# Crowsinc/LiveVisionKit

Measured on AMD Instinct MI355X. Metric: stabilized frames/sec (one 4K YUV420 stream per GPU, steady state), higher is better.
Workload: dtype f32

## Files before the change

### include/lvk_hip.h

```cpp
#ifndef LVK_HIP_H
#define LVK_HIP_H

#include <stdint.h>
#include <stddef.h>

#ifdef __cplusplus
extern "C" {
#endif

#define LVK_HIP_OK              0
#define LVK_HIP_ERR_ARG        -1
#define LVK_HIP_ERR_RUNTIME    -2
#define LVK_HIP_ERR_NO_DEVICE  -3

typedef struct lvk_hip_ctx lvk_hip_ctx;


int  lvk_hip_ctx_create(int device, lvk_hip_ctx** out);
int  lvk_hip_ctx_create_on_stream(int device, void* hip_stream, lvk_hip_ctx** out);
void lvk_hip_ctx_destroy(lvk_hip_ctx* ctx);
int  lvk_hip_sync(lvk_hip_ctx* ctx);
void* lvk_hip_stream(lvk_hip_ctx* ctx);
const char* lvk_hip_last_error(lvk_hip_ctx* ctx);
const char* lvk_hip_version(void);
#define LVK_HIP_ABI_VERSION 12
int  lvk_hip_abi_version(void);
int  lvk_hip_device_count(void);
int  lvk_hip_device_usable(int device);

int  lvk_hip_ctx_wait(lvk_hip_ctx* ctx, lvk_hip_ctx* producer);

int lvk_hip_malloc(lvk_hip_ctx* ctx, size_t bytes, void** d_ptr);
int lvk_hip_free(lvk_hip_ctx* ctx, void* d_ptr);
int lvk_hip_trim(lvk_hip_ctx* ctx);
int lvk_hip_upload(lvk_hip_ctx* ctx, void* d_dst, const void* h_src, size_t bytes);
int lvk_hip_download(lvk_hip_ctx* ctx, void* h_dst, const void* d_src, size_t bytes);

int  lvk_hip_host_malloc(lvk_hip_ctx* ctx, size_t bytes, void** h_ptr);
int  lvk_hip_host_free(lvk_hip_ctx* ctx, void* h_ptr);


int lvk_hip_remap_homography(lvk_hip_ctx* ctx,
                             const void* d_src, int src_step, int src_rows, int src_cols,
                             void* d_dst, int dst_step, int dst_rows, int dst_cols,
                             int off_x, int off_y, const float H[9], const uint8_t bg[3], int yuv);

int lvk_hip_remap_mesh(lvk_hip_ctx* ctx,
                       const void* d_src, int src_step, int src_rows, int src_cols,
                       void* d_dst, int dst_step,
                       const float* mesh, int mesh_rows, int mesh_cols, const uint8_t bg[3], int yuv);

int lvk_hip_remap_map(lvk_hip_ctx* ctx, const void* d_src, int src_step, int rows, int cols, void* d_dst, int dst_step,
                      const void* d_map, int map_step, const uint8_t bg[3], int yuv);

#define LVK_REMAP_EXACT 0
#define LVK_REMAP_1LSB  1
int lvk_hip_set_remap_precision(lvk_hip_ctx* ctx, int precision);
int lvk_hip_get_remap_precision(lvk_hip_ctx* ctx);

int lvk_hip_upscale(lvk_hip_ctx* ctx, const void* d_src, int src_step, int src_rows, int src_cols,
                    void* d_dst, int dst_step, int dst_rows, int dst_cols, int yuv);

int lvk_hip_sharpen(lvk_hip_ctx* ctx, const void* d_src, int src_step, int rows, int cols, void* d_dst, int dst_step, float sharpness);

typedef struct lvk_camera_params { double fx, fy, cx, cy, k1, k2, p1, p2, k3; } lvk_camera_params;
int lvk_hip_lens_map_create(lvk_hip_ctx* ctx, const lvk_camera_params* params, int rows, int cols, void** d_map, int view_xywh[4]);
int lvk_hip_lens_map_destroy(lvk_hip_ctx* ctx, void* d_map);
int lvk_hip_warpmesh_apply_lens(lvk_hip_ctx* ctx, const void* d_src, int src_step, int rows, int cols, void* d_dst, int dst_step,
                                const float* mesh, int mesh_rows, int mesh_cols, const uint8_t bg[3], int yuv, const lvk_camera_params* lens);
int lvk_hip_lens_undistort_points(lvk_hip_ctx* ctx, const lvk_camera_params* params, int rows, int cols, double sx, double sy,
                                  const float* pts, int n, float* out);

int lvk_hip_warpmesh_apply_yuv420(lvk_hip_ctx* ctx, const void* d_src, int src_step, int rows, int cols,
                                  void* o_y, int oy_step, void* o_u, int ou_step, void* o_v, int ov_step, int nv12,
                                  const float* mesh, int mesh_rows, int mesh_cols, const uint8_t bg[3]);

int lvk_hip_warpmesh_apply(lvk_hip_ctx* ctx,
                           const void* d_src, int src_step, int rows, int cols,
                           void* d_dst, int dst_step,
                           const float* mesh, int mesh_rows, int mesh_cols, const uint8_t bg[3], int yuv);

int lvk_hip_ingest_yuv420(lvk_hip_ctx* ctx, const void* d_y, int y_step, const void* d_u, int u_step, const void* d_v, int v_step, int nv12,
                          int rows, int cols, void* d_dst, int dst_step);
int lvk_hip_egress_yuv420(lvk_hip_ctx* ctx, const void* d_src, int src_step, int rows, int cols,
                          void* d_y, int y_step, void* d_u, int u_step, void* d_v, int v_step, int nv12);

#define LVK_VIDEO_FORMAT_I420 1
#define LVK_VIDEO_FORMAT_NV12 2
#define LVK_VIDEO_FORMAT_YVYU 3
#define LVK_VIDEO_FORMAT_YUY2 4
#define LVK_VIDEO_FORMAT_UYVY 5
#define LVK_VIDEO_FORMAT_RGBA 6
#define LVK_VIDEO_FORMAT_BGRA 7
#define LVK_VIDEO_FORMAT_BGRX 8
#define LVK_VIDEO_FORMAT_Y800 9
#define LVK_VIDEO_FORMAT_I444 10
#define LVK_VIDEO_FORMAT_BGR3 11
#define LVK_VIDEO_FORMAT_I422 12
#define LVK_VIDEO_FORMAT_I40A 13
#define LVK_VIDEO_FORMAT_I42A 14
#define LVK_VIDEO_FORMAT_YUVA 15
#define LVK_VIDEO_FORMAT_AYUV 16
int lvk_hip_ingest_obs(lvk_hip_ctx* ctx, int video_format, const void* const d_planes[3], const int steps[3], int rows, int cols, void* d_dst, int dst_step);
int lvk_hip_egress_obs(lvk_hip_ctx* ctx, int video_format, const void* d_src, int src_step, int rows, int cols, void* const d_planes[3], const int steps[3]);
int lvk_hip_obs_frame_format(int video_format);

typedef struct lvk_stab_settings
{
    int detection_width, detection_height;
    int detection_regions_x, detection_regions_y;
    int force_detection;
    float max_feature_density, min_feature_density, accumulation_rate;
    int track_local_motions;
    float temporal_smoothing, local_smoothing;
    int min_motion_samples;
    float acceptance_threshold, uniformity_threshold;
    int predictive_samples;
    float corrective_limit_x, corrective_limit_y;
    float smoothing_steps, response_rate;
    int motion_width, motion_height;
    float background[3];
    int crop_to_stable_region, stabilize_output;
    float min_scene_quality, min_tracking_quality;
} lvk_stab_settings;

typedef struct lvk_stab_stats
{
    float tracking_stability;
    float scene_quality, trust;
    float distribution;
    int n_detected, n_matched, n_tracked, frame_delay;
    double smoothing_factor;
    double homography[9];
} lvk_stab_stats;

#define LVK_FORMAT_BGR 0
#define LVK_FORMAT_BGRA 1
#define LVK_FORMAT_RGB 2
#define LVK_FORMAT_RGBA 3
#define LVK_FORMAT_YUV 4
#define LVK_FORMAT_GRAY 5

typedef struct lvk_hip_stab lvk_hip_stab;

void lvk_stab_default_settings(lvk_stab_settings* s);
int  lvk_hip_stab_create(lvk_hip_ctx* ctx, const lvk_stab_settings* settings, lvk_hip_stab** out);
void lvk_hip_stab_destroy(lvk_hip_stab* stab);
int  lvk_hip_stab_configure(lvk_hip_stab* stab, const lvk_stab_settings* settings);
int  lvk_hip_stab_restart(lvk_hip_stab* stab);
int  lvk_hip_stab_draw_trackers(lvk_hip_stab* stab);
int  lvk_hip_stab_draw_motion_mesh(lvk_hip_stab* stab);
int  lvk_hip_draw_grid(lvk_hip_ctx* ctx, void* d_dst, int dst_step, int rows, int cols, int grid_w, int grid_h, const uint8_t colour[3], int thickness);
int  lvk_hip_draw_crosses(lvk_hip_ctx* ctx, void* d_dst, int dst_step, int rows, int cols, const float* pts_xy, int n,
                          float scale_x, float scale_y, const uint8_t colour[3], int cross_size, int thickness);
int  lvk_hip_draw_points(lvk_hip_ctx* ctx, void* d_dst, int dst_step, int rows, int cols, const float* pts_xy, int n, float scale_x, float scale_y,
                         const uint8_t colour[3], int point_size);
int  lvk_hip_draw_rect(lvk_hip_ctx* ctx, void* d_dst, int dst_step, int rows, int cols, const int rect_xywh[4], const uint8_t colour[3], int thickness);
int  lvk_hip_draw_text(lvk_hip_ctx* ctx, void* d_dst, int dst_step, int rows, int cols, const char* text, int x, int y, const uint8_t colour[3],
                       int scale, int thickness);
int  lvk_hip_stab_set_lens(lvk_hip_stab* stab, const lvk_camera_params* params);
int  lvk_hip_stab_reset_context(lvk_hip_stab* stab);
int  lvk_hip_stab_ready(const lvk_hip_stab* stab);
int  lvk_hip_stab_frame_delay(const lvk_hip_stab* stab);
int  lvk_hip_stab_stable_region(const lvk_hip_stab* stab, int rows, int cols, int rect_xywh[4]);

typedef struct lvk_frame_info { int rows, cols, format; } lvk_frame_info;
int  lvk_hip_stab_next_output(const lvk_hip_stab* stab, int rows, int cols, int format, lvk_frame_info* out);
int  lvk_hip_stab_push(lvk_hip_stab* stab, const void* d_frame, int step, int rows, int cols, uint64_t timestamp, int format,
                       void* d_out, int out_step, int out_rows, int* produced, uint64_t* out_timestamp, const void** released,
                       lvk_frame_info* emitted);

int  lvk_hip_stab_push_yuv420(lvk_hip_stab* stab, const void* d_y, int y_step, const void* d_u, int u_step, const void* d_v, int v_step, int nv12,
                              int rows, int cols, uint64_t timestamp,
                              void* o_y, int oy_step, void* o_u, int ou_step, void* o_v, int ov_step, int o_rows,
                              int* produced, uint64_t* out_timestamp, lvk_frame_info* emitted);
int  lvk_hip_stab_push_obs(lvk_hip_stab* stab, int video_format, const void* const d_planes[3], const int steps[3], int rows, int cols, uint64_t timestamp,
                           void* const o_planes[3], const int o_steps[3], int o_rows, int* produced, uint64_t* out_timestamp, lvk_frame_info* emitted);

int  lvk_hip_stab_push_yuv420_host(lvk_hip_stab* stab, const void* h_y, int y_step, const void* h_u, int u_step, const void* h_v, int v_step, int nv12,
                                   int rows, int cols, uint64_t timestamp,
                                   void* oh_y, int oy_step, void* oh_u, int ou_step, void* oh_v, int ov_step, int o_rows,
                                   int* produced, uint64_t* out_timestamp, lvk_frame_info* emitted);
int  lvk_hip_stab_push_obs_host(lvk_hip_stab* stab, int video_format,
                                const void* const h_planes[3], const int steps[3], int rows, int cols, uint64_t timestamp,
                                void* const oh_planes[3], const int o_steps[3], int o_rows,
                                int* produced, uint64_t* out_timestamp, lvk_frame_info* emitted);
int  lvk_hip_stab_prefetch_yuv420_host(lvk_hip_stab* stab, const void* h_y, int y_step, const void* h_u, int u_step, const void* h_v, int v_step,
                                       int nv12, int rows, int cols);
int  lvk_hip_stab_prefetch_cancel(lvk_hip_stab* stab);
int  lvk_hip_stab_set_overlap(lvk_hip_stab* stab, int enable);
int  lvk_hip_stab_set_bulk_context(lvk_hip_stab* stab, lvk_hip_ctx* bulk);
void* lvk_hip_stab_output_stream(lvk_hip_stab* stab);
int  lvk_hip_stab_set_remap_precision(lvk_hip_stab* stab, int precision);
int  lvk_hip_stab_get_remap_precision(const lvk_hip_stab* stab);


typedef struct lvk_deblock_settings
{
    uint32_t detection_levels;
    uint32_t block_size;
    uint32_t filter_size;
    float filter_scaling;
} lvk_deblock_settings;

typedef struct lvk_hip_deblock lvk_hip_deblock;

void lvk_hip_deblock_default_settings(lvk_deblock_settings* s);
int  lvk_hip_deblock_create(lvk_hip_ctx* ctx, const lvk_deblock_settings* settings, lvk_hip_deblock** out);
int  lvk_hip_deblock_configure(lvk_hip_deblock* deb, const lvk_deblock_settings* settings);
void lvk_hip_deblock_destroy(lvk_hip_deblock* deb);
int  lvk_hip_deblock_apply(lvk_hip_deblock* deb, void* d_frame, int step, int rows, int cols, int format, int region_xywh[4]);
int  lvk_hip_deblock_draw_influence(const lvk_hip_deblock* deb, void* d_frame, int step, int rows, int cols, int format);
int  lvk_hip_deblock_filter_region(const lvk_hip_deblock* deb, int region_xywh[4]);

int  lvk_hip_cas(lvk_hip_ctx* ctx, const void* d_src, int src_step, int rows, int cols, int format, void* d_dst, int dst_step, float sharpness);

int  lvk_hip_reformat(lvk_hip_ctx* ctx, const void* d_src, int src_step, int rows, int cols, int src_format, void* d_dst, int dst_step,
                      int dst_format);

int  lvk_hip_fsr_easu(lvk_hip_ctx* ctx, const void* d_src, int src_step, int rows, int cols, int format, const int region_xywh[4], void* d_dst,
                      int dst_step, int out_rows, int out_cols);
int  lvk_hip_fsr_geometry(int rows, int cols, int out_rows, int out_cols, float multiplier, int maintain_aspect_ratio, const int crop_ltrb[4],
                          int region_xywh[4], int out_rows_cols[2], int* skip);
int  lvk_hip_text_size(const char* text, int scale, int thickness, int wh[2], int* baseline);



int  lvk_hip_stab_prefetch(lvk_hip_stab* stab, const void* d_frame, int step, int rows, int cols, int format);
int  lvk_hip_stab_prefetch_yuv420(lvk_hip_stab* stab, const void* d_y, int y_step, const void* d_u, int u_step, const void* d_v, int v_step,
                                  int nv12, int rows, int cols);
long long lvk_hip_stab_lookahead_frames(lvk_hip_stab* stab);

int lvk_hip_remap_homography_gray(lvk_hip_ctx* ctx, const void* d_src, int src_step, int src_rows, int src_cols,
                                  void* d_dst, int dst_step, int dst_rows, int dst_cols, int off_x, int off_y, const float H[9], uint8_t bg);
int lvk_hip_remap_mesh_gray(lvk_hip_ctx* ctx, const void* d_src, int src_step, int src_rows, int src_cols, void* d_dst, int dst_step,
                            const float* mesh, int mesh_rows, int mesh_cols, uint8_t bg);
int lvk_hip_remap_map_gray(lvk_hip_ctx* ctx, const void* d_src, int src_step, int rows, int cols, void* d_dst, int dst_step,
                           const void* d_map, int map_step, uint8_t bg);
int lvk_hip_warpmesh_apply_gray(lvk_hip_ctx* ctx, const void* d_src, int src_step, int rows, int cols, void* d_dst, int dst_step,
                                const float* mesh, int mesh_rows, int mesh_cols, uint8_t bg);
int lvk_hip_warpmesh_apply_lens_gray(lvk_hip_ctx* ctx, const void* d_src, int src_step, int rows, int cols, void* d_dst, int dst_step,
                                     const float* mesh, int mesh_rows, int mesh_cols, uint8_t bg, const lvk_camera_params* lens);
int  lvk_hip_stab_push_gray(lvk_hip_stab* stab, const void* d_frame, int step, int rows, int cols, uint64_t timestamp,
                            void* d_out, int out_step, int out_rows, int* produced, uint64_t* out_timestamp, const void** released,
                            lvk_frame_info* emitted);
int  lvk_hip_stab_push_gray_host(lvk_hip_stab* stab, const void* h_frame, int step, int rows, int cols, uint64_t timestamp,
                                 void* oh_out, int out_step, int out_rows, int* produced, uint64_t* out_timestamp, lvk_frame_info* emitted);

int lvk_hip_remap_homography_c4(lvk_hip_ctx* ctx, const void* d_src, int src_step, int src_rows, int src_cols,
                                void* d_dst, int dst_step, int dst_rows, int dst_cols, int off_x, int off_y, const float H[9], const uint8_t bg[4]);
int lvk_hip_remap_mesh_c4(lvk_hip_ctx* ctx, const void* d_src, int src_step, int src_rows, int src_cols, void* d_dst, int dst_step,
                          const float* mesh, int mesh_rows, int mesh_cols, const uint8_t bg[4]);
int lvk_hip_remap_map_c4(lvk_hip_ctx* ctx, const void* d_src, int src_step, int rows, int cols, void* d_dst, int dst_step,
                         const void* d_map, int map_step, const uint8_t bg[4]);
int lvk_hip_warpmesh_apply_c4(lvk_hip_ctx* ctx, const void* d_src, int src_step, int rows, int cols, void* d_dst, int dst_step,
                              const float* mesh, int mesh_rows, int mesh_cols, const uint8_t bg[4]);
int lvk_hip_warpmesh_apply_lens_c4(lvk_hip_ctx* ctx, const void* d_src, int src_step, int rows, int cols, void* d_dst, int dst_step,
                                   const float* mesh, int mesh_rows, int mesh_cols, const uint8_t bg[4], const lvk_camera_params* lens);
int  lvk_hip_stab_set_background_alpha(lvk_hip_stab* stab, int alpha);
int  lvk_hip_stab_push_c4(lvk_hip_stab* stab, const void* d_frame, int step, int rows, int cols, uint64_t timestamp, int format,
                          void* d_out, int out_step, int out_rows, int* produced, uint64_t* out_timestamp, const void** released,
                          lvk_frame_info* emitted);
int  lvk_hip_stab_push_c4_host(lvk_hip_stab* stab, const void* h_frame, int step, int rows, int cols, uint64_t timestamp, int format,
                               void* oh_out, int out_step, int out_rows, int* produced, uint64_t* out_timestamp, lvk_frame_info* emitted);

int lvk_hip_upscale_gray(lvk_hip_ctx* ctx, const void* d_src, int src_step, int src_rows, int src_cols, void* d_dst, int dst_step, int dst_rows, int dst_cols);
int lvk_hip_upscale_c4(lvk_hip_ctx* ctx, const void* d_src, int src_step, int src_rows, int src_cols, void* d_dst, int dst_step, int dst_rows, int dst_cols);
int lvk_hip_sharpen_gray(lvk_hip_ctx* ctx, const void* d_src, int src_step, int rows, int cols, void* d_dst, int dst_step, float sharpness);
int lvk_hip_sharpen_c4(lvk_hip_ctx* ctx, const void* d_src, int src_step, int rows, int cols, void* d_dst, int dst_step, float sharpness);

int lvk_hip_cas_gray(lvk_hip_ctx* ctx, const void* d_src, int src_step, int rows, int cols, void* d_dst, int dst_step, float sharpness);
int lvk_hip_fsr_easu_gray(lvk_hip_ctx* ctx, const void* d_src, int src_step, int rows, int cols, const int region_xywh[4],
                          void* d_dst, int dst_step, int out_rows, int out_cols);
int lvk_hip_fsr_easu_gray_path(int rw, int rh, int out_rows, int out_cols);


#define LVK_SCHED_PUSH_FREE_RUNNING   0
#define LVK_SCHED_PUSH_SYNCHRONISED   1
#define LVK_SCHED_INGEST_ON_TRACKER   2
#define LVK_SCHED_INGEST_ON_BULK      3
#define LVK_SCHED_INGEST_INLINE       4
#define LVK_SCHED_REMAP_PERSISTENT    5
#define LVK_SCHED_REMAP_FULL          6
#define LVK_SCHED_WAIT_SIGNAL_WORD    7
#define LVK_SCHED_WAIT_EVENT          8
#define LVK_SCHED_WAIT_WORD_TIMEOUT   9
#define LVK_SCHED_COUNT              10
int  lvk_hip_stab_schedule_counters(lvk_hip_stab* stab, long long out[LVK_SCHED_COUNT], int reset);

int  lvk_hip_stab_get_stats(const lvk_hip_stab* stab, lvk_stab_stats* out);
int  lvk_hip_stab_detector_frames(const lvk_hip_stab* stab, long long* on_device, long long* on_host);
int  lvk_hip_stab_get_meshes(const lvk_hip_stab* stab, float* motion, float* correction, int cap_floats);
int  lvk_hip_stab_get_features(const lvk_hip_stab* stab, float* xy_resp_age, int cap);


#define LVK_STAGE_DOWNSCALE 0
#define LVK_STAGE_PYRAMID   1
#define LVK_STAGE_FAST      2
#define LVK_STAGE_PYRLK     3
#define LVK_STAGE_MOTION    4
#define LVK_STAGE_REMAP     5
#define LVK_STAGE_INGEST    6
#define LVK_STAGE_EGRESS    7
#define LVK_STAGE_COUNT     8
int  lvk_hip_stab_set_profiling(lvk_hip_stab* stab, int enable);
int  lvk_hip_stab_get_profile(lvk_hip_stab* stab, double total_ms[LVK_STAGE_COUNT], long long launches[LVK_STAGE_COUNT]);

int lvk_hip_native_rcp(lvk_hip_ctx* ctx, const float* d_in, float* d_out, size_t n);

typedef struct lvk_hip_mesh_solver lvk_hip_mesh_solver;
int  lvk_hip_mesh_solver_create(lvk_hip_ctx* ctx, int cols, int rows, float gen_region_w, float gen_region_h,
                                float temporal_smoothing, float local_smoothing, int max_points, lvk_hip_mesh_solver** out);
void lvk_hip_mesh_solver_destroy(lvk_hip_mesh_solver* solver);
int  lvk_hip_mesh_solver_reset(lvk_hip_mesh_solver* solver);
int  lvk_hip_mesh_solver_solve(lvk_hip_mesh_solver* solver, const float* tracked, const float* matched, int n, float region_w, float region_h,
                               float temporal_now, float threshold, uint8_t* inliers, float* offsets);

int lvk_hip_luma_area_resize(lvk_hip_ctx* ctx, const void* d_src, int src_step, int pix_stride, int channel,
                             int srows, int scols, void* d_dst, int dst_step, int drows, int dcols);

int lvk_hip_pyr_down(lvk_hip_ctx* ctx, const void* d_src, int src_step, int rows, int cols, void* d_dst, int dst_step);
int lvk_hip_scharr(lvk_hip_ctx* ctx, const void* d_src, int src_step, int rows, int cols, void* d_dst);

int lvk_hip_build_pyramid(lvk_hip_ctx* ctx, const void* d_img, int step, int rows, int cols, int max_level, int win_w, int win_h,
                          uint8_t* levels, int16_t* derivs, int* level_rows, int* level_cols);

int lvk_hip_fast_detect(lvk_hip_ctx* ctx, const void* d_img, int step, int rows, int cols,
                        const int* regions, int nregions, uint32_t* out, int cap, int* counts);

int lvk_hip_pyrlk(lvk_hip_ctx* ctx, const void* d_prev, int prev_step, const void* d_next, int next_step, int rows, int cols,
                  const float* prev_pts, int n, float* next_pts, uint8_t* status,
                  int win_w, int win_h, int max_level, int max_count, double epsilon, double min_eig_threshold);

int lvk_hip_estimate_global_motion(lvk_hip_ctx* ctx, const float* pts1, const float* pts2, int n, double threshold,
                                   double region_w, double region_h, int full_homography, double H[9], uint8_t* mask);

int lvk_hip_estimate_global_motion_lo(lvk_hip_ctx* ctx, const float* pts1, const float* pts2, int n, double threshold,
                                      double region_w, double region_h, int full_homography, int lo_mode, double H[9], uint8_t* mask,
                                      int lo_info[2]);

int lvk_hip_fast_filter(lvk_hip_ctx* ctx, const float* prev, const float* matched, const uint8_t* status, int n, float* out_prev, float* out_matched);

#define LVK_TRACK_CHAIN_GUARD 64
#define LVK_TRACK_CHAIN_FILL  0xA5
typedef struct lvk_track_chain_desc
{
    const float* prev; const float* matched; const uint8_t* status; const float* und;
    const void* d_prev_img; int prev_step; const void* d_next_img; int next_step; int rows, cols;
    int win_w, win_h, max_level, max_count; double epsilon, min_eig;
    const lvk_camera_params* lens; int lens_rows, lens_cols; double lens_sx, lens_sy;
    int n_bound, count_on_device, n_word;
    int full, model_on_device, full_word;
    int separate_compact, host_signal;
    double threshold; int region_w, region_h;
} lvk_track_chain_desc;
typedef struct lvk_track_chain_result
{
    double H[9]; int rc, signalled, count_dev, count_host;
    uint8_t* mask; float* pairs_dev; float* mirror_matched; uint8_t* mirror_status;
    float* next_pts; uint8_t* flow_status; float* flow_und;
} lvk_track_chain_result;
int lvk_hip_track_chain(lvk_hip_ctx* ctx, const lvk_track_chain_desc* desc, lvk_track_chain_result* result);

int lvk_hip_deblock_get_grid(lvk_hip_deblock* deb, uint8_t* mean, uint8_t* grid, float* keep_block, int capacity, int extent_xy[2]);


int lvk_hip_cas_const(float sharpness, float* peak);

int lvk_hip_cvt_code_target(int code, int src_format, int dcn);

int lvk_hip_fsr_easu_const(int rw, int rh, int W, int H, int ow, int oh, float con[16]);

int lvk_hip_fsr_easu_path(int rw, int rh, int out_rows, int out_cols);

enum
{
    LVK_AREA_PATH_FAST_DW_8x8_C3_BGR = 0, LVK_AREA_PATH_FAST_DW_8x8_C3_RGB = 1, LVK_AREA_PATH_FAST_DW_4x4_C3_BGR = 2, LVK_AREA_PATH_FAST_DW_4x4_C3_RGB = 3,
    LVK_AREA_PATH_FAST_DW_8x8_C3 = 4, LVK_AREA_PATH_FAST_DW_4x4_C3 = 5, LVK_AREA_PATH_FAST_DW_8x8_C1 = 6, LVK_AREA_PATH_FAST_DW_4x4_C1 = 7,
    LVK_AREA_PATH_FAST = 8, LVK_AREA_PATH_TILE_4 = 9, LVK_AREA_PATH_TILE_8 = 10, LVK_AREA_PATH_TAPS_4 = 11, LVK_AREA_PATH_TAPS_8 = 12,
    LVK_AREA_PATH_GENERAL = 13, LVK_AREA_PATH_ENLARGE = 14, LVK_AREA_PATH_COUNT = 15
};
int lvk_hip_area_resize_path(lvk_hip_ctx* ctx, const void* d_src, int src_step, int pix_stride, int channel,
                             int srows, int scols, int drows, int dcols);

int lvk_hip_remap_map_yuv420(lvk_hip_ctx* ctx, const void* d_src, int src_step, int rows, int cols,
                             void* o_y, int oy_step, void* o_u, int ou_step, void* o_v, int ov_step, int nv12,
                             const void* d_map, int map_step, const uint8_t bg[3]);
typedef struct lvk_hip_lens lvk_hip_lens;
int  lvk_hip_lens_create(lvk_hip_ctx* ctx, const lvk_camera_params* profile , int test_mode, lvk_hip_lens** out);
int  lvk_hip_lens_configure(lvk_hip_lens* lens, const lvk_camera_params* profile, int test_mode);
void lvk_hip_lens_destroy(lvk_hip_lens* lens);
int  lvk_hip_lens_view(lvk_hip_lens* lens, int rows, int cols, int view_xywh[4]);
int  lvk_hip_lens_apply(lvk_hip_lens* lens, void* d_src, int src_step, int rows, int cols, int format, void* d_dst, int dst_step);
int  lvk_hip_lens_apply_gray(lvk_hip_lens* lens, const void* d_src, int src_step, int rows, int cols, void* d_dst, int dst_step);
int  lvk_hip_lens_apply_c4(lvk_hip_lens* lens, const void* d_src, int src_step, int rows, int cols, int format, void* d_dst, int dst_step);
int  lvk_hip_lens_apply_yuv420(lvk_hip_lens* lens, const void* d_y, int y_step, const void* d_u, int u_step, const void* d_v, int v_step,
                               void* o_y, int oy_step, void* o_u, int ou_step, void* o_v, int ov_step, int rows, int cols, int nv12);

#ifdef __cplusplus
}
#endif

#include "lvk_hip_scaling_420.h"
#include "lvk_hip_deblock_420.h"
#include "lvk_hip_deblock_px.h"
#endif
```

### livevisionkit_amd/_native.py

```python
import ctypes
import os

_HERE = os.path.dirname(os.path.abspath(__file__))
LIB_PATH = os.environ.get("LVK_HIP_LIB") or os.path.join(_HERE, "liblvk_hip.so")

_c = ctypes
_P = _c.c_void_p
_SIG = {
    "lvk_hip_ctx_create": (_c.c_int, [_c.c_int, _c.POINTER(_P)]),
    "lvk_hip_ctx_create_on_stream": (_c.c_int, [_c.c_int, _P, _c.POINTER(_P)]),
    "lvk_hip_ctx_destroy": (None, [_P]),
    "lvk_hip_sync": (_c.c_int, [_P]),
    "lvk_hip_stream": (_P, [_P]),
    "lvk_hip_last_error": (_c.c_char_p, [_P]),
    "lvk_hip_version": (_c.c_char_p, []),
    "lvk_hip_abi_version": (_c.c_int, []),
    "lvk_hip_device_count": (_c.c_int, []),
    "lvk_hip_device_usable": (_c.c_int, [_c.c_int]),
    "lvk_hip_malloc": (_c.c_int, [_P, _c.c_size_t, _c.POINTER(_P)]),
    "lvk_hip_free": (_c.c_int, [_P, _P]),
    "lvk_hip_trim": (_c.c_int, [_P]),
    "lvk_hip_ctx_wait": (_c.c_int, [_P, _P]),
    "lvk_hip_upload": (_c.c_int, [_P, _P, _P, _c.c_size_t]),
    "lvk_hip_download": (_c.c_int, [_P, _P, _P, _c.c_size_t]),
    "lvk_hip_remap_homography": (_c.c_int, [_P, _P, _c.c_int, _c.c_int, _c.c_int, _P, _c.c_int, _c.c_int, _c.c_int,
                                            _c.c_int, _c.c_int, _c.POINTER(_c.c_float), _c.POINTER(_c.c_uint8), _c.c_int]),
    "lvk_hip_remap_mesh": (_c.c_int, [_P, _P, _c.c_int, _c.c_int, _c.c_int, _P, _c.c_int,
                                      _c.POINTER(_c.c_float), _c.c_int, _c.c_int, _c.POINTER(_c.c_uint8), _c.c_int]),
    "lvk_hip_remap_map": (_c.c_int, [_P, _P, _c.c_int, _c.c_int, _c.c_int, _P, _c.c_int, _P, _c.c_int, _c.POINTER(_c.c_uint8), _c.c_int]),
    "lvk_hip_remap_homography_gray": (_c.c_int, [_P, _P, _c.c_int, _c.c_int, _c.c_int, _P, _c.c_int, _c.c_int, _c.c_int,
                                                 _c.c_int, _c.c_int, _c.POINTER(_c.c_float), _c.c_uint8]),
    "lvk_hip_remap_mesh_gray": (_c.c_int, [_P, _P, _c.c_int, _c.c_int, _c.c_int, _P, _c.c_int, _c.POINTER(_c.c_float), _c.c_int, _c.c_int, _c.c_uint8]),
    "lvk_hip_remap_map_gray": (_c.c_int, [_P, _P, _c.c_int, _c.c_int, _c.c_int, _P, _c.c_int, _P, _c.c_int, _c.c_uint8]),
    "lvk_hip_warpmesh_apply_gray": (_c.c_int, [_P, _P, _c.c_int, _c.c_int, _c.c_int, _P, _c.c_int, _c.POINTER(_c.c_float), _c.c_int, _c.c_int, _c.c_uint8]),
    "lvk_hip_warpmesh_apply_lens_gray": (_c.c_int, [_P, _P, _c.c_int, _c.c_int, _c.c_int, _P, _c.c_int, _c.POINTER(_c.c_float), _c.c_int, _c.c_int, _c.c_uint8, _P]),
    "lvk_hip_stab_push_gray": (_c.c_int, [_P, _P, _c.c_int, _c.c_int, _c.c_int, _c.c_uint64, _P, _c.c_int, _c.c_int,
                                          _c.POINTER(_c.c_int), _c.POINTER(_c.c_uint64), _c.POINTER(_P), _P]),
    "lvk_hip_stab_push_gray_host": (_c.c_int, [_P, _P, _c.c_int, _c.c_int, _c.c_int, _c.c_uint64, _P, _c.c_int, _c.c_int,
                                               _c.POINTER(_c.c_int), _c.POINTER(_c.c_uint64), _P]),
    "lvk_hip_set_remap_precision": (_c.c_int, [_P, _c.c_int]),
    "lvk_hip_get_remap_precision": (_c.c_int, [_P]),
    "lvk_hip_stab_set_remap_precision": (_c.c_int, [_P, _c.c_int]),
    "lvk_hip_stab_get_remap_precision": (_c.c_int, [_P]),
    "lvk_hip_remap_homography_c4": (_c.c_int, [_P, _P, _c.c_int, _c.c_int, _c.c_int, _P, _c.c_int, _c.c_int, _c.c_int,
                                               _c.c_int, _c.c_int, _c.POINTER(_c.c_float), _c.POINTER(_c.c_uint8)]),
    "lvk_hip_remap_mesh_c4": (_c.c_int, [_P, _P, _c.c_int, _c.c_int, _c.c_int, _P, _c.c_int, _c.POINTER(_c.c_float), _c.c_int, _c.c_int, _c.POINTER(_c.c_uint8)]),
    "lvk_hip_remap_map_c4": (_c.c_int, [_P, _P, _c.c_int, _c.c_int, _c.c_int, _P, _c.c_int, _P, _c.c_int, _c.POINTER(_c.c_uint8)]),
    "lvk_hip_warpmesh_apply_c4": (_c.c_int, [_P, _P, _c.c_int, _c.c_int, _c.c_int, _P, _c.c_int, _c.POINTER(_c.c_float), _c.c_int, _c.c_int, _c.POINTER(_c.c_uint8)]),
    "lvk_hip_warpmesh_apply_lens_c4": (_c.c_int, [_P, _P, _c.c_int, _c.c_int, _c.c_int, _P, _c.c_int, _c.POINTER(_c.c_float), _c.c_int, _c.c_int, _c.POINTER(_c.c_uint8), _P]),
    "lvk_hip_stab_set_background_alpha": (_c.c_int, [_P, _c.c_int]),
    "lvk_hip_stab_push_c4": (_c.c_int, [_P, _P, _c.c_int, _c.c_int, _c.c_int, _c.c_uint64, _c.c_int, _P, _c.c_int, _c.c_int,
                                        _c.POINTER(_c.c_int), _c.POINTER(_c.c_uint64), _c.POINTER(_P), _P]),
    "lvk_hip_stab_push_c4_host": (_c.c_int, [_P, _P, _c.c_int, _c.c_int, _c.c_int, _c.c_uint64, _c.c_int, _P, _c.c_int, _c.c_int,
                                             _c.POINTER(_c.c_int), _c.POINTER(_c.c_uint64), _P]),
    "lvk_hip_upscale": (_c.c_int, [_P, _P, _c.c_int, _c.c_int, _c.c_int, _P, _c.c_int, _c.c_int, _c.c_int, _c.c_int]),
    "lvk_hip_sharpen": (_c.c_int, [_P, _P, _c.c_int, _c.c_int, _c.c_int, _P, _c.c_int, _c.c_float]),
    "lvk_hip_upscale_gray": (_c.c_int, [_P, _P, _c.c_int, _c.c_int, _c.c_int, _P, _c.c_int, _c.c_int, _c.c_int]),
    "lvk_hip_upscale_c4": (_c.c_int, [_P, _P, _c.c_int, _c.c_int, _c.c_int, _P, _c.c_int, _c.c_int, _c.c_int]),
    "lvk_hip_sharpen_gray": (_c.c_int, [_P, _P, _c.c_int, _c.c_int, _c.c_int, _P, _c.c_int, _c.c_float]),
    "lvk_hip_sharpen_c4": (_c.c_int, [_P, _P, _c.c_int, _c.c_int, _c.c_int, _P, _c.c_int, _c.c_float]),
    "lvk_hip_native_rcp": (_c.c_int, [_P, _P, _P, _c.c_size_t]),
    "lvk_hip_mesh_solver_create": (_c.c_int, [_P, _c.c_int, _c.c_int, _c.c_float, _c.c_float, _c.c_float, _c.c_float, _c.c_int, _c.POINTER(_P)]),
    "lvk_hip_mesh_solver_destroy": (None, [_P]),
    "lvk_hip_mesh_solver_reset": (_c.c_int, [_P]),
    "lvk_hip_mesh_solver_solve": (_c.c_int, [_P, _c.POINTER(_c.c_float), _c.POINTER(_c.c_float), _c.c_int, _c.c_float, _c.c_float, _c.c_float, _c.c_float,
                                             _c.POINTER(_c.c_uint8), _c.POINTER(_c.c_float)]),
    "lvk_hip_lens_map_create": (_c.c_int, [_P, _P, _c.c_int, _c.c_int, _c.POINTER(_P), _c.POINTER(_c.c_int)]),
    "lvk_hip_lens_map_destroy": (_c.c_int, [_P, _P]),
    "lvk_hip_warpmesh_apply_lens": (_c.c_int, [_P, _P, _c.c_int, _c.c_int, _c.c_int, _P, _c.c_int, _c.POINTER(_c.c_float), _c.c_int, _c.c_int, _c.POINTER(_c.c_uint8), _c.c_int, _P]),
    "lvk_hip_lens_undistort_points": (_c.c_int, [_P, _P, _c.c_int, _c.c_int, _c.c_double, _c.c_double, _c.POINTER(_c.c_float), _c.c_int, _c.POINTER(_c.c_float)]),
    "lvk_hip_stab_set_lens": (_c.c_int, [_P, _P]),
    "lvk_hip_stab_output_stream": (_P, [_P]),
    "lvk_hip_fast_filter": (_c.c_int, [_P, _c.POINTER(_c.c_float), _c.POINTER(_c.c_float), _c.POINTER(_c.c_uint8), _c.c_int, _c.POINTER(_c.c_float), _c.POINTER(_c.c_float)]),
    "lvk_hip_stab_draw_trackers": (_c.c_int, [_P]),
    "lvk_hip_stab_draw_motion_mesh": (_c.c_int, [_P]),
    "lvk_hip_draw_grid": (_c.c_int, [_P, _P, _c.c_int, _c.c_int, _c.c_int, _c.c_int, _c.c_int, _c.POINTER(_c.c_uint8), _c.c_int]),
    "lvk_hip_draw_crosses": (_c.c_int, [_P, _P, _c.c_int, _c.c_int, _c.c_int, _c.POINTER(_c.c_float), _c.c_int, _c.c_float, _c.c_float,
                                        _c.POINTER(_c.c_uint8), _c.c_int, _c.c_int]),
    "lvk_hip_draw_points": (_c.c_int, [_P, _P, _c.c_int, _c.c_int, _c.c_int, _c.POINTER(_c.c_float), _c.c_int, _c.c_float, _c.c_float,
                                       _c.POINTER(_c.c_uint8), _c.c_int]),
    "lvk_hip_draw_rect": (_c.c_int, [_P, _P, _c.c_int, _c.c_int, _c.c_int, _c.POINTER(_c.c_int), _c.POINTER(_c.c_uint8), _c.c_int]),
    "lvk_hip_draw_text": (_c.c_int, [_P, _P, _c.c_int, _c.c_int, _c.c_int, _c.c_char_p, _c.c_int, _c.c_int, _c.POINTER(_c.c_uint8), _c.c_int, _c.c_int]),
    "lvk_hip_text_size": (_c.c_int, [_c.c_char_p, _c.c_int, _c.c_int, _c.POINTER(_c.c_int), _c.POINTER(_c.c_int)]),
    "lvk_hip_warpmesh_apply_yuv420": (_c.c_int, [_P, _P, _c.c_int, _c.c_int, _c.c_int, _P, _c.c_int, _P, _c.c_int, _P, _c.c_int, _c.c_int,
                                                 _c.POINTER(_c.c_float), _c.c_int, _c.c_int, _c.POINTER(_c.c_uint8)]),
    "lvk_hip_warpmesh_apply": (_c.c_int, [_P, _P, _c.c_int, _c.c_int, _c.c_int, _P, _c.c_int,
                                          _c.POINTER(_c.c_float), _c.c_int, _c.c_int, _c.POINTER(_c.c_uint8), _c.c_int]),
    "lvk_hip_luma_area_resize": (_c.c_int, [_P, _P, _c.c_int, _c.c_int, _c.c_int, _c.c_int, _c.c_int, _P, _c.c_int, _c.c_int, _c.c_int]),
    "lvk_hip_pyr_down": (_c.c_int, [_P, _P, _c.c_int, _c.c_int, _c.c_int, _P, _c.c_int]),
    "lvk_hip_scharr": (_c.c_int, [_P, _P, _c.c_int, _c.c_int, _c.c_int, _P]),
    "lvk_hip_build_pyramid": (_c.c_int, [_P, _P, _c.c_int, _c.c_int, _c.c_int, _c.c_int, _c.c_int, _c.c_int,
                                         _c.POINTER(_c.c_uint8), _c.POINTER(_c.c_int16), _c.POINTER(_c.c_int), _c.POINTER(_c.c_int)]),
    "lvk_hip_fast_detect": (_c.c_int, [_P, _P, _c.c_int, _c.c_int, _c.c_int, _c.POINTER(_c.c_int), _c.c_int,
                                       _c.POINTER(_c.c_uint32), _c.c_int, _c.POINTER(_c.c_int)]),
    "lvk_hip_pyrlk": (_c.c_int, [_P, _P, _c.c_int, _P, _c.c_int, _c.c_int, _c.c_int, _c.POINTER(_c.c_float), _c.c_int,
                                 _c.POINTER(_c.c_float), _c.POINTER(_c.c_uint8), _c.c_int, _c.c_int, _c.c_int, _c.c_int,
                                 _c.c_double, _c.c_double]),
    "lvk_hip_ingest_yuv420": (_c.c_int, [_P, _P, _c.c_int, _P, _c.c_int, _P, _c.c_int, _c.c_int, _c.c_int, _c.c_int, _P, _c.c_int]),
    "lvk_hip_egress_yuv420": (_c.c_int, [_P, _P, _c.c_int, _c.c_int, _c.c_int, _P, _c.c_int, _P, _c.c_int, _P, _c.c_int, _c.c_int]),
    "lvk_hip_ingest_obs": (_c.c_int, [_P, _c.c_int, _P * 3, _c.c_int * 3, _c.c_int, _c.c_int, _P, _c.c_int]),
    "lvk_hip_egress_obs": (_c.c_int, [_P, _c.c_int, _P, _c.c_int, _c.c_int, _c.c_int, _P * 3, _c.c_int * 3]),
    "lvk_hip_obs_frame_format": (_c.c_int, [_c.c_int]),
    "lvk_hip_estimate_global_motion": (_c.c_int, [_P, _c.POINTER(_c.c_float), _c.POINTER(_c.c_float), _c.c_int, _c.c_double,
                                                  _c.c_double, _c.c_double, _c.c_int, _c.POINTER(_c.c_double), _c.POINTER(_c.c_uint8)]),
    "lvk_hip_estimate_global_motion_lo": (_c.c_int, [_P, _c.POINTER(_c.c_float), _c.POINTER(_c.c_float), _c.c_int, _c.c_double,
                                                     _c.c_double, _c.c_double, _c.c_int, _c.c_int, _c.POINTER(_c.c_double), _c.POINTER(_c.c_uint8),
                                                     _c.POINTER(_c.c_int)]),
    "lvk_hip_track_chain": (_c.c_int, [_P, _P, _P]),
    "lvk_stab_default_settings": (None, [_P]),
    "lvk_hip_stab_create": (_c.c_int, [_P, _P, _c.POINTER(_P)]),
    "lvk_hip_stab_destroy": (None, [_P]),
    "lvk_hip_stab_configure": (_c.c_int, [_P, _P]),
    "lvk_hip_stab_restart": (_c.c_int, [_P]),
    "lvk_hip_stab_reset_context": (_c.c_int, [_P]),
    "lvk_hip_stab_ready": (_c.c_int, [_P]),
    "lvk_hip_stab_frame_delay": (_c.c_int, [_P]),
    "lvk_hip_stab_stable_region": (_c.c_int, [_P, _c.c_int, _c.c_int, _c.POINTER(_c.c_int)]),
    "lvk_hip_stab_next_output": (_c.c_int, [_P, _c.c_int, _c.c_int, _c.c_int, _P]),
    "lvk_hip_stab_push": (_c.c_int, [_P, _P, _c.c_int, _c.c_int, _c.c_int, _c.c_uint64, _c.c_int, _P, _c.c_int, _c.c_int,
                                     _c.POINTER(_c.c_int), _c.POINTER(_c.c_uint64), _c.POINTER(_P), _P]),
    "lvk_hip_stab_push_yuv420": (_c.c_int, [_P, _P, _c.c_int, _P, _c.c_int, _P, _c.c_int, _c.c_int, _c.c_int, _c.c_int, _c.c_uint64,
                                            _P, _c.c_int, _P, _c.c_int, _P, _c.c_int, _c.c_int, _c.POINTER(_c.c_int), _c.POINTER(_c.c_uint64), _P]),
    "lvk_hip_stab_push_obs": (_c.c_int, [_P, _c.c_int, _P * 3, _c.c_int * 3, _c.c_int, _c.c_int, _c.c_uint64, _P * 3, _c.c_int * 3, _c.c_int,
                                         _c.POINTER(_c.c_int), _c.POINTER(_c.c_uint64), _P]),
    "lvk_hip_stab_push_yuv420_host": (_c.c_int, [_P, _P, _c.c_int, _P, _c.c_int, _P, _c.c_int, _c.c_int, _c.c_int, _c.c_int, _c.c_uint64,
                                            _P, _c.c_int, _P, _c.c_int, _P, _c.c_int, _c.c_int, _c.POINTER(_c.c_int), _c.POINTER(_c.c_uint64), _P]),
    "lvk_hip_stab_push_obs_host": (_c.c_int, [_P, _c.c_int, _P * 3, _c.c_int * 3, _c.c_int, _c.c_int, _c.c_uint64, _P * 3, _c.c_int * 3, _c.c_int,
                                              _c.POINTER(_c.c_int), _c.POINTER(_c.c_uint64), _P]),
    "lvk_hip_stab_prefetch_yuv420_host": (_c.c_int, [_P, _P, _c.c_int, _P, _c.c_int, _P, _c.c_int, _c.c_int, _c.c_int, _c.c_int]),
    "lvk_hip_stab_prefetch_cancel": (_c.c_int, [_P]),
    "lvk_hip_stab_prefetch": (_c.c_int, [_P, _P, _c.c_int, _c.c_int, _c.c_int, _c.c_int]),
    "lvk_hip_stab_prefetch_yuv420": (_c.c_int, [_P, _P, _c.c_int, _P, _c.c_int, _P, _c.c_int, _c.c_int, _c.c_int, _c.c_int]),
    "lvk_hip_stab_lookahead_frames": (_c.c_longlong, [_P]),
    "lvk_hip_stab_schedule_counters": (_c.c_int, [_P, _c.POINTER(_c.c_longlong), _c.c_int]),
    "lvk_hip_stab_detector_frames": (_c.c_int, [_P, _c.POINTER(_c.c_longlong), _c.POINTER(_c.c_longlong)]),
    "lvk_hip_host_malloc": (_c.c_int, [_P, _c.c_size_t, _c.POINTER(_P)]),
    "lvk_hip_host_free": (_c.c_int, [_P, _P]),
    "lvk_hip_stab_get_stats": (_c.c_int, [_P, _P]),
    "lvk_hip_stab_get_meshes": (_c.c_int, [_P, _c.POINTER(_c.c_float), _c.POINTER(_c.c_float), _c.c_int]),
    "lvk_hip_stab_get_features": (_c.c_int, [_P, _c.POINTER(_c.c_float), _c.c_int]),
    "lvk_hip_stab_set_overlap": (_c.c_int, [_P, _c.c_int]),
    "lvk_hip_stab_set_bulk_context": (_c.c_int, [_P, _P]),
    "lvk_hip_stab_set_profiling": (_c.c_int, [_P, _c.c_int]),
    "lvk_hip_stab_get_profile": (_c.c_int, [_P, _c.POINTER(_c.c_double), _c.POINTER(_c.c_longlong)]),
    "lvk_hip_deblock_default_settings": (None, [_P]),
    "lvk_hip_deblock_create": (_c.c_int, [_P, _P, _c.POINTER(_P)]),
    "lvk_hip_deblock_configure": (_c.c_int, [_P, _P]),
    "lvk_hip_deblock_destroy": (None, [_P]),
    "lvk_hip_deblock_apply": (_c.c_int, [_P, _P, _c.c_int, _c.c_int, _c.c_int, _c.c_int, _c.POINTER(_c.c_int)]),
    "lvk_hip_deblock_draw_influence": (_c.c_int, [_P, _P, _c.c_int, _c.c_int, _c.c_int, _c.c_int]),
    "lvk_hip_deblock_filter_region": (_c.c_int, [_P, _c.POINTER(_c.c_int)]),
    "lvk_hip_deblock_get_grid": (_c.c_int, [_P, _c.POINTER(_c.c_uint8), _c.POINTER(_c.c_uint8), _c.POINTER(_c.c_float), _c.c_int, _c.POINTER(_c.c_int)]),
    "lvk_hip_cas": (_c.c_int, [_P, _P, _c.c_int, _c.c_int, _c.c_int, _c.c_int, _P, _c.c_int, _c.c_float]),
    "lvk_hip_cas_const": (_c.c_int, [_c.c_float, _c.POINTER(_c.c_float)]),
    "lvk_hip_reformat": (_c.c_int, [_P, _P, _c.c_int, _c.c_int, _c.c_int, _c.c_int, _P, _c.c_int, _c.c_int]),
    "lvk_hip_cvt_code_target": (_c.c_int, [_c.c_int, _c.c_int, _c.c_int]),
    "lvk_hip_fsr_easu": (_c.c_int, [_P, _P, _c.c_int, _c.c_int, _c.c_int, _c.c_int, _c.POINTER(_c.c_int), _P, _c.c_int, _c.c_int, _c.c_int]),
    "lvk_hip_fsr_geometry": (_c.c_int, [_c.c_int, _c.c_int, _c.c_int, _c.c_int, _c.c_float, _c.c_int, _c.POINTER(_c.c_int), _c.POINTER(_c.c_int),
                                        _c.POINTER(_c.c_int), _c.POINTER(_c.c_int)]),
    "lvk_hip_fsr_easu_const": (_c.c_int, [_c.c_int, _c.c_int, _c.c_int, _c.c_int, _c.c_int, _c.c_int, _c.POINTER(_c.c_float)]),
    "lvk_hip_fsr_easu_path": (_c.c_int, [_c.c_int, _c.c_int, _c.c_int, _c.c_int]),
    "lvk_hip_cas_gray": (_c.c_int, [_P, _P, _c.c_int, _c.c_int, _c.c_int, _P, _c.c_int, _c.c_float]),
    "lvk_hip_fsr_easu_gray": (_c.c_int, [_P, _P, _c.c_int, _c.c_int, _c.c_int, _c.POINTER(_c.c_int), _P, _c.c_int, _c.c_int, _c.c_int]),
    "lvk_hip_fsr_easu_gray_path": (_c.c_int, [_c.c_int, _c.c_int, _c.c_int, _c.c_int]),
    "lvk_hip_area_resize_path": (_c.c_int, [_P, _P, _c.c_int, _c.c_int, _c.c_int, _c.c_int, _c.c_int, _c.c_int, _c.c_int]),
    "lvk_hip_remap_map_yuv420": (_c.c_int, [_P, _P, _c.c_int, _c.c_int, _c.c_int, _P, _c.c_int, _P, _c.c_int, _P, _c.c_int, _c.c_int,
                                            _P, _c.c_int, _c.POINTER(_c.c_uint8)]),
    "lvk_hip_lens_create": (_c.c_int, [_P, _P, _c.c_int, _c.POINTER(_P)]),
    "lvk_hip_lens_configure": (_c.c_int, [_P, _P, _c.c_int]),
    "lvk_hip_lens_destroy": (None, [_P]),
    "lvk_hip_lens_view": (_c.c_int, [_P, _c.c_int, _c.c_int, _c.POINTER(_c.c_int)]),
    "lvk_hip_lens_apply": (_c.c_int, [_P, _P, _c.c_int, _c.c_int, _c.c_int, _c.c_int, _P, _c.c_int]),
    "lvk_hip_lens_apply_gray": (_c.c_int, [_P, _P, _c.c_int, _c.c_int, _c.c_int, _P, _c.c_int]),
    "lvk_hip_lens_apply_c4": (_c.c_int, [_P, _P, _c.c_int, _c.c_int, _c.c_int, _c.c_int, _P, _c.c_int]),
    "lvk_hip_lens_apply_yuv420": (_c.c_int, [_P, _P, _c.c_int, _P, _c.c_int, _P, _c.c_int, _P, _c.c_int, _P, _c.c_int, _P, _c.c_int,
                                             _c.c_int, _c.c_int, _c.c_int]),
}

_SIG_DEBLOCK_PX = {
    "lvk_hip_deblock_apply_gray": (_c.c_int, [_P, _P, _c.c_int, _c.c_int, _c.c_int, _c.POINTER(_c.c_int)]),
    "lvk_hip_deblock_apply_c4": (_c.c_int, [_P, _P, _c.c_int, _c.c_int, _c.c_int, _c.c_int, _c.POINTER(_c.c_int)]),
}

_SIG_DEBLOCK_420 = {
    "lvk_hip_deblock_apply_yuv420": (_c.c_int, [_P, _P, _c.c_int, _P, _c.c_int, _P, _c.c_int, _P, _c.c_int, _P, _c.c_int, _P, _c.c_int,
                                                _c.c_int, _c.c_int, _c.c_int, _c.POINTER(_c.c_int)]),
}

_SIG_SCALING_420 = {
    "lvk_hip_scale_yuv420": (_c.c_int, [_P, _P, _c.c_int, _P, _c.c_int, _P, _c.c_int, _c.c_int, _c.c_int,
                                        _P, _c.c_int, _P, _c.c_int, _P, _c.c_int, _c.c_int, _c.c_int, _c.c_int, _c.c_float]),
}

_lib = None


def symbols():
    return sorted(_SIG.keys())


def symbols_deblock_px():
    return sorted(_SIG_DEBLOCK_PX.keys())


def symbols_deblock_420():
    return sorted(_SIG_DEBLOCK_420.keys())


def symbols_scaling_420():
    return sorted(_SIG_SCALING_420.keys())


def load():
    global _lib
    if _lib is not None:
        return _lib
    if not os.path.exists(LIB_PATH):
        raise RuntimeError(
            f"{LIB_PATH} is missing: build it with `python -c 'import __graft_entry__ as g; g.build()'` "
            "(or `make -C livevisionkit_amd/csrc`). There is no CPU fallback.")
    import torch
    lib = ctypes.CDLL(LIB_PATH, mode=ctypes.RTLD_GLOBAL)
    for name, (res, args) in {**_SIG, **_SIG_DEBLOCK_PX, **_SIG_DEBLOCK_420, **_SIG_SCALING_420}.items():
        fn = getattr(lib, name)
        fn.restype = res
        fn.argtypes = args
    _lib = lib
    return lib
```

### livevisionkit_amd/context.py

```python
import ctypes

import numpy as np

from . import _native


class LvkHipError(RuntimeError):
    pass


def _f32(a):
    a = np.ascontiguousarray(a, dtype=np.float32)
    return a, a.ctypes.data_as(ctypes.POINTER(ctypes.c_float))


def _u8x3(bg):
    a = np.ascontiguousarray(bg, dtype=np.uint8).reshape(3)
    return a, a.ctypes.data_as(ctypes.POINTER(ctypes.c_uint8))


def _u8x4(bg):
    a = np.ascontiguousarray(bg, dtype=np.uint8).reshape(4)
    return a, a.ctypes.data_as(ctypes.POINTER(ctypes.c_uint8))


def _planes420_empty(rows, cols, nv12, device):
    import torch
    y = torch.empty((rows, cols), dtype=torch.uint8, device=device)
    u = torch.empty((rows // 2, cols // 2, 2) if nv12 else (rows // 2, cols // 2), dtype=torch.uint8, device=device)
    return (y, u) if nv12 else (y, u, torch.empty_like(u))


def _planes420_args(planes, nv12):
    a = []
    for p in planes[:2 if nv12 else 3]:
        a += [p.data_ptr(), p.stride(0)]
    return a + ([None, 0] if nv12 else [])


TRACK_CHAIN_GUARD = 64
TRACK_CHAIN_FILL = 0xA5


class TrackChainDesc(ctypes.Structure):
    _fields_ = [("prev", ctypes.POINTER(ctypes.c_float)), ("matched", ctypes.POINTER(ctypes.c_float)), ("status", ctypes.POINTER(ctypes.c_uint8)),
                ("und", ctypes.POINTER(ctypes.c_float)),
                ("d_prev_img", ctypes.c_void_p), ("prev_step", ctypes.c_int), ("d_next_img", ctypes.c_void_p), ("next_step", ctypes.c_int),
                ("rows", ctypes.c_int), ("cols", ctypes.c_int),
                ("win_w", ctypes.c_int), ("win_h", ctypes.c_int), ("max_level", ctypes.c_int), ("max_count", ctypes.c_int),
                ("epsilon", ctypes.c_double), ("min_eig", ctypes.c_double),
                ("lens", ctypes.c_void_p), ("lens_rows", ctypes.c_int), ("lens_cols", ctypes.c_int), ("lens_sx", ctypes.c_double), ("lens_sy", ctypes.c_double),
                ("n_bound", ctypes.c_int), ("count_on_device", ctypes.c_int), ("n_word", ctypes.c_int),
                ("full", ctypes.c_int), ("model_on_device", ctypes.c_int), ("full_word", ctypes.c_int),
                ("separate_compact", ctypes.c_int), ("host_signal", ctypes.c_int),
                ("threshold", ctypes.c_double), ("region_w", ctypes.c_int), ("region_h", ctypes.c_int)]


class TrackChainResult(ctypes.Structure):
    _fields_ = [("H", ctypes.c_double * 9), ("rc", ctypes.c_int), ("signalled", ctypes.c_int), ("count_dev", ctypes.c_int), ("count_host", ctypes.c_int),
                ("mask", ctypes.POINTER(ctypes.c_uint8)), ("pairs_dev", ctypes.POINTER(ctypes.c_float)), ("mirror_matched", ctypes.POINTER(ctypes.c_float)),
                ("mirror_status", ctypes.POINTER(ctypes.c_uint8)),
                ("next_pts", ctypes.POINTER(ctypes.c_float)), ("flow_status", ctypes.POINTER(ctypes.c_uint8)), ("flow_und", ctypes.POINTER(ctypes.c_float))]

REMAP_EXACT, REMAP_1LSB = 0, 1


def _remap_precision(precision):
    if isinstance(precision, str):
        return {"exact": REMAP_EXACT, "1lsb": REMAP_1LSB}.get(precision.lower(), -1)
    return int(precision)


class Context:

    def __init__(self, device=0, stream=None):
        import torch
        if not torch.cuda.is_available():
            raise LvkHipError("no GPU visible: the lvk HIP path has no CPU fallback")
        self.lib = _native.load()
        self.device = device
        torch.cuda.set_device(device)
        self._torch_stream = stream if stream is not None else torch.cuda.current_stream(device)
        handle = ctypes.c_void_p()
        rc = self.lib.lvk_hip_ctx_create_on_stream(device, ctypes.c_void_p(self._torch_stream.cuda_stream), ctypes.byref(handle))
        if rc != 0:
            raise LvkHipError(f"lvk_hip_ctx_create failed ({rc}): {self.lib.lvk_hip_last_error(None).decode()}")
        self.handle = handle

    def close(self):
        if getattr(self, "handle", None):
            self.lib.lvk_hip_ctx_destroy(self.handle)
            self.handle = None

    def __del__(self):
        try:
            self.close()
        except Exception:
            pass

    def _check(self, rc):
        if rc != 0:
            raise LvkHipError(f"lvk_hip call failed ({rc}): {self.lib.lvk_hip_last_error(self.handle).decode()}")

    def sync(self):
        self._check(self.lib.lvk_hip_sync(self.handle))

    def set_remap_precision(self, precision):
        self._check(self.lib.lvk_hip_set_remap_precision(self.handle, _remap_precision(precision)))

    @property
    def remap_precision(self):
        return self.lib.lvk_hip_get_remap_precision(self.handle)

    def remap_homography(self, src, H, bg=(255, 0, 255), yuv=True, out=None, dst_size=None, offset=(0, 0)):
        import torch
        rows, cols = src.shape[0], src.shape[1]
        drows, dcols = dst_size if dst_size is not None else (rows, cols)
        if out is None:
            out = torch.empty((drows, dcols, 3), dtype=torch.uint8, device=src.device)
        Ha, Hp = _f32(np.asarray(H, dtype=np.float32).reshape(9))
        bga, bgp = _u8x3(bg)
        self._check(self.lib.lvk_hip_remap_homography(
            self.handle, src.data_ptr(), src.stride(0), rows, cols, out.data_ptr(), out.stride(0), drows, dcols,
            offset[0], offset[1], Hp, bgp, 1 if yuv else 0))
        return out

    def remap_mesh(self, src, mesh, bg=(255, 0, 255), yuv=True, out=None):
        import torch
        rows, cols = src.shape[0], src.shape[1]
        if out is None:
            out = torch.empty((rows, cols, 3), dtype=torch.uint8, device=src.device)
        m = np.ascontiguousarray(mesh, dtype=np.float32)
        ma, mp = _f32(m)
        bga, bgp = _u8x3(bg)
        self._check(self.lib.lvk_hip_remap_mesh(
            self.handle, src.data_ptr(), src.stride(0), rows, cols, out.data_ptr(), out.stride(0),
            mp, m.shape[0], m.shape[1], bgp, 1 if yuv else 0))
        return out

    def warpmesh_apply(self, src, mesh, bg=(255, 0, 255), yuv=True, out=None):
        import torch
        rows, cols = src.shape[0], src.shape[1]
        if out is None:
            out = torch.empty((rows, cols, 3), dtype=torch.uint8, device=src.device)
        m = np.ascontiguousarray(mesh, dtype=np.float32)
        ma, mp = _f32(m)
        bga, bgp = _u8x3(bg)
        self._check(self.lib.lvk_hip_warpmesh_apply(
            self.handle, src.data_ptr(), src.stride(0), rows, cols, out.data_ptr(), out.stride(0),
            mp, m.shape[0], m.shape[1], bgp, 1 if yuv else 0))
        return out

    def _px_out(self, sfx, src, out, shape=None):
        import torch
        if sfx == "_gray" and src.dim() != 2:
            raise ValueError("a one-channel frame is a [rows, cols] uint8 tensor")
        if sfx == "_c4" and (src.dim() != 3 or src.shape[2] != 4):
            raise ValueError("a four-channel frame is a [rows, cols, 4] uint8 tensor")
        return out if out is not None else torch.empty(tuple(shape or src.shape[:2]) + tuple(src.shape[2:]), dtype=torch.uint8, device=src.device)

    def _px_call(self, name, sfx, src, out, bg, mid, tail=(), shape=None):
        out = self._px_out(sfx, src, out, shape)
        bga, bgp = (None, int(bg)) if sfx == "_gray" else _u8x4(bg)
        self._check(getattr(self.lib, "lvk_hip_" + name + sfx)(self.handle, src.data_ptr(), src.stride(0), src.shape[0], src.shape[1], out.data_ptr(), out.stride(0),
                                                               *mid, bgp, *tail))
        return out

    def _px_homography(self, sfx, src, H, bg, out, dst_size, offset):
        drows, dcols = dst_size if dst_size is not None else tuple(src.shape[:2])
        Ha, Hp = _f32(np.asarray(H, dtype=np.float32).reshape(9))
        return self._px_call("remap_homography", sfx, src, out, bg, (drows, dcols, offset[0], offset[1], Hp), shape=(drows, dcols))

    def _px_mesh(self, name, sfx, src, mesh, bg, out, lens=None):
        ma, mp = _f32(mesh)
        tail = () if lens is None else ((ctypes.c_double * 9)(*[float(v) for v in lens]),)
        return self._px_call(name, sfx, src, out, bg, (mp, ma.shape[0], ma.shape[1]), tail)

    def _px_map(self, sfx, src, offsets, bg, out):
        return self._px_call("remap_map", sfx, src, out, bg, (offsets.data_ptr(), offsets.stride(0) * 4))

    def remap_homography_gray(self, src, H, bg=0, out=None, dst_size=None, offset=(0, 0)):
        return self._px_homography("_gray", src, H, bg, out, dst_size, offset)

    def remap_mesh_gray(self, src, mesh, bg=0, out=None):
        return self._px_mesh("remap_mesh", "_gray", src, mesh, bg, out)

    def remap_map_gray(self, src, offsets, bg=0, out=None):
        return self._px_map("_gray", src, offsets, bg, out)

    def warpmesh_apply_gray(self, src, mesh, bg=0, out=None, lens=None):
        return self._px_mesh("warpmesh_apply" if lens is None else "warpmesh_apply_lens", "_gray", src, mesh, bg, out, lens)

    def remap_homography_c4(self, src, H, bg=(255, 0, 255, 255), out=None, dst_size=None, offset=(0, 0)):
        return self._px_homography("_c4", src, H, bg, out, dst_size, offset)

    def remap_mesh_c4(self, src, mesh, bg=(255, 0, 255, 255), out=None):
        return self._px_mesh("remap_mesh", "_c4", src, mesh, bg, out)

    def remap_map_c4(self, src, offsets, bg=(255, 0, 255, 255), out=None):
        return self._px_map("_c4", src, offsets, bg, out)

    def warpmesh_apply_c4(self, src, mesh, bg=(255, 0, 255, 255), out=None):
        return self._px_mesh("warpmesh_apply", "_c4", src, mesh, bg, out)

    def warpmesh_apply_lens_c4(self, src, mesh, lens, bg=(255, 0, 255, 255), out=None):
        return self._px_mesh("warpmesh_apply_lens", "_c4", src, mesh, bg, out, lens)

    def luma_area_resize(self, frame, drows, dcols, channel=0, out=None):
        import torch
        pix = frame.shape[2] if frame.dim() == 3 else 1
        if out is None:
            out = torch.empty((drows, dcols), dtype=torch.uint8, device=frame.device)
        self._check(self.lib.lvk_hip_luma_area_resize(self.handle, frame.data_ptr(), frame.stride(0), pix, channel,
                                                      frame.shape[0], frame.shape[1], out.data_ptr(), out.stride(0), drows, dcols))
        return out

    def area_resize_path(self, frame, drows, dcols, channel=0):
        pix = frame.shape[2] if frame.dim() == 3 else 1
        path = self.lib.lvk_hip_area_resize_path(self.handle, frame.data_ptr(), frame.stride(0), pix, channel, frame.shape[0], frame.shape[1], drows, dcols)
        self._check(min(path, 0))
        return path

    def pyr_down(self, img, out=None):
        import torch
        if out is None:
            out = torch.empty(((img.shape[0] + 1) // 2, (img.shape[1] + 1) // 2), dtype=torch.uint8, device=img.device)
        self._check(self.lib.lvk_hip_pyr_down(self.handle, img.data_ptr(), img.stride(0), img.shape[0], img.shape[1],
                                              out.data_ptr(), out.stride(0)))
        return out

    def scharr(self, img, out=None):
        import torch
        if out is None:
            out = torch.empty((img.shape[0], img.shape[1], 2), dtype=torch.int16, device=img.device)
        self._check(self.lib.lvk_hip_scharr(self.handle, img.data_ptr(), img.stride(0), img.shape[0], img.shape[1], out.data_ptr()))
        return out

    def build_pyramid(self, img, max_level=3, win=(11, 11)):
        rows, cols = img.shape
        lv = np.zeros(rows * cols * 2, np.uint8); dv = np.zeros(rows * cols * 4, np.int16)
        lr = np.zeros(8, np.int32); lc = np.zeros(8, np.int32)
        n = self.lib.lvk_hip_build_pyramid(self.handle, img.data_ptr(), img.stride(0), rows, cols, max_level, win[0], win[1],
                                           lv.ctypes.data_as(ctypes.POINTER(ctypes.c_uint8)), dv.ctypes.data_as(ctypes.POINTER(ctypes.c_int16)),
                                           lr.ctypes.data_as(ctypes.POINTER(ctypes.c_int)), lc.ctypes.data_as(ctypes.POINTER(ctypes.c_int)))
        self._check(min(n, 0))
        out, lo, do = [], 0, 0
        for i in range(n):
            r, c = int(lr[i]), int(lc[i])
            out.append((lv[lo:lo + r * c].reshape(r, c).copy(), dv[do:do + r * c * 2].reshape(r, c, 2).copy()))
            lo += r * c; do += r * c * 2
        return out

    def fast_detect(self, img, regions, cap=None):
        rg = np.ascontiguousarray(regions, dtype=np.int32).reshape(-1, 6)
        n = rg.shape[0]
        cap = cap or int(max(1, (rg[:, 2] * rg[:, 3]).max()))
        out = np.zeros((n, cap), np.uint32)
        counts = np.zeros(n, np.int32)
        self._check(self.lib.lvk_hip_fast_detect(self.handle, img.data_ptr(), img.stride(0), img.shape[0], img.shape[1],
                                                 rg.ctypes.data_as(ctypes.POINTER(ctypes.c_int)), n,
                                                 out.ctypes.data_as(ctypes.POINTER(ctypes.c_uint32)), cap,
                                                 counts.ctypes.data_as(ctypes.POINTER(ctypes.c_int))))
        res = []
        for i in range(n):
            e = out[i, :min(cap, counts[i])]
            res.append(np.stack([e & 0xFFF, (e >> 12) & 0xFFF, e >> 24], axis=1).astype(np.int32))
        return res, counts

    def pyrlk(self, prev, nxt, pts, win=(11, 11), max_level=3, max_count=5, epsilon=0.01, min_eig=1e-4):
        pts = np.ascontiguousarray(pts, np.float32).reshape(-1, 2)
        out = np.zeros_like(pts)
        st = np.zeros(len(pts), np.uint8)
        self._check(self.lib.lvk_hip_pyrlk(self.handle, prev.data_ptr(), prev.stride(0), nxt.data_ptr(), nxt.stride(0),
                                           prev.shape[0], prev.shape[1],
                                           pts.ctypes.data_as(ctypes.POINTER(ctypes.c_float)), len(pts),
                                           out.ctypes.data_as(ctypes.POINTER(ctypes.c_float)),
                                           st.ctypes.data_as(ctypes.POINTER(ctypes.c_uint8)),
                                           win[0], win[1], max_level, max_count, float(epsilon), float(min_eig)))
        return out, st

    def estimate_global_motion(self, p1, p2, threshold, region=(480, 270), full_homography=True):
        p1 = np.ascontiguousarray(p1, np.float32).reshape(-1, 2); p2 = np.ascontiguousarray(p2, np.float32).reshape(-1, 2)
        H = np.zeros(9, np.float64); mask = np.zeros(len(p1), np.uint8)
        rc = self.lib.lvk_hip_estimate_global_motion(self.handle, p1.ctypes.data_as(ctypes.POINTER(ctypes.c_float)),
                                                     p2.ctypes.data_as(ctypes.POINTER(ctypes.c_float)), len(p1), float(threshold),
                                                     float(region[0]), float(region[1]), 1 if full_homography else 0,
                                                     H.ctypes.data_as(ctypes.POINTER(ctypes.c_double)),
                                                     mask.ctypes.data_as(ctypes.POINTER(ctypes.c_uint8)))
        if rc in (-1, -2, -3):
            self._check(rc)
        return rc, H.reshape(3, 3), mask

    def estimate_global_motion_lo(self, p1, p2, threshold, lo_mode, region=(480, 270), full_homography=True):
        p1 = np.ascontiguousarray(p1, np.float32).reshape(-1, 2); p2 = np.ascontiguousarray(p2, np.float32).reshape(-1, 2)
        H = np.zeros(9, np.float64); mask = np.zeros(len(p1), np.uint8); info = (ctypes.c_int * 2)(-1, -1)
        rc = self.lib.lvk_hip_estimate_global_motion_lo(self.handle, p1.ctypes.data_as(ctypes.POINTER(ctypes.c_float)),
                                                        p2.ctypes.data_as(ctypes.POINTER(ctypes.c_float)), len(p1), float(threshold),
                                                        float(region[0]), float(region[1]), 1 if full_homography else 0, int(lo_mode),
                                                        H.ctypes.data_as(ctypes.POINTER(ctypes.c_double)),
                                                        mask.ctypes.data_as(ctypes.POINTER(ctypes.c_uint8)), info)
        if rc in (-1, -2, -3):
            self._check(rc)
        return rc, H.reshape(3, 3), mask, info[0], info[1]

    def ingest_yuv420(self, y, u, v=None, out=None):
        import torch
        rows, cols = y.shape
        if out is None:
            out = torch.empty((rows, cols, 3), dtype=torch.uint8, device=y.device)
        nv12 = v is None
        self._check(self.lib.lvk_hip_ingest_yuv420(self.handle, *_planes420_args((y, u, v), nv12), 1 if nv12 else 0, rows, cols, out.data_ptr(), out.stride(0)))
        return out

    def egress_yuv420(self, frame, nv12=False, out=None):
        rows, cols = frame.shape[:2]
        if out is None:
            out = _planes420_empty(rows, cols, nv12, frame.device)
        y, u, v = out if not nv12 else (out[0], out[1], None)
        self._check(self.lib.lvk_hip_egress_yuv420(self.handle, frame.data_ptr(), frame.stride(0), rows, cols, *_planes420_args((y, u, v), nv12), 1 if nv12 else 0))
        return (y, u) if nv12 else (y, u, v)

    VIDEO_FORMATS = {"I420": 1, "NV12": 2, "YVYU": 3, "YUY2": 4, "UYVY": 5, "RGBA": 6, "BGRA": 7, "BGRX": 8, "Y800": 9, "I444": 10, "BGR3": 11,
                     "I422": 12, "I40A": 13, "I42A": 14, "YUVA": 15, "AYUV": 16}

    def _obs_args(self, planes):
        import ctypes as c
        ptrs = (c.c_void_p * 3)(*[p.data_ptr() for p in planes] + [None] * (3 - len(planes)))
        steps = (c.c_int * 3)(*[p.stride(0) for p in planes] + [0] * (3 - len(planes)))
        return ptrs, steps

    def ingest_obs(self, fmt, planes, out=None):
        import torch
        rows, cols = planes[0].shape[:2]
        if out is None:
            out = torch.empty((rows, cols) if fmt == "Y800" else (rows, cols, 3), dtype=torch.uint8, device=planes[0].device)
        ptrs, steps = self._obs_args(planes)
        self._check(self.lib.lvk_hip_ingest_obs(self.handle, self.VIDEO_FORMATS[fmt], ptrs, steps, rows, cols, out.data_ptr(), out.stride(0)))
        return out

    def egress_obs(self, fmt, frame, planes):
        rows, cols = frame.shape[:2]
        ptrs, steps = self._obs_args(planes)
        self._check(self.lib.lvk_hip_egress_obs(self.handle, self.VIDEO_FORMATS[fmt], frame.data_ptr(), frame.stride(0), rows, cols, ptrs, steps))
        return planes

    def obs_frame_format(self, fmt):
        return self.lib.lvk_hip_obs_frame_format(self.VIDEO_FORMATS[fmt] if isinstance(fmt, str) else int(fmt))

    def remap_map(self, src, offsets, bg=(255, 0, 255), yuv=True, out=None):
        import torch
        rows, cols = src.shape[:2]
        if out is None:
            out = torch.empty_like(src)
        bga, bgp = _u8x3(bg)
        self._check(self.lib.lvk_hip_remap_map(self.handle, src.data_ptr(), src.stride(0), rows, cols, out.data_ptr(), out.stride(0),
                                               offsets.data_ptr(), offsets.stride(0) * 4, bgp, 1 if yuv else 0))
        return out

    def remap_map_yuv420(self, src, offsets, bg=(255, 0, 255), nv12=False, out=None):
        rows, cols = src.shape[0], src.shape[1]
        out = _planes420_empty(rows, cols, nv12, src.device) if out is None else tuple(out)
        bga, bgp = _u8x3(bg)
        self._check(self.lib.lvk_hip_remap_map_yuv420(self.handle, src.data_ptr(), src.stride(0), rows, cols, *_planes420_args(out, nv12), 1 if nv12 else 0,
                                                      offsets.data_ptr(), offsets.stride(0) * 4, bgp))
        return out

    def upscale(self, src, size, yuv=True, out=None):
        import torch
        rows, cols = src.shape[:2]
        if out is None:
            out = torch.empty((int(size[1]), int(size[0]), 3), dtype=torch.uint8, device=src.device)
        self._check(self.lib.lvk_hip_upscale(self.handle, src.data_ptr(), src.stride(0), rows, cols,
                                             out.data_ptr(), out.stride(0), out.shape[0], out.shape[1], 1 if yuv else 0))
        return out

    def sharpen(self, src, sharpness=0.7, out=None):
        import torch
        rows, cols = src.shape[:2]
        if out is None:
            out = torch.empty_like(src)
        self._check(self.lib.lvk_hip_sharpen(self.handle, src.data_ptr(), src.stride(0), rows, cols, out.data_ptr(), out.stride(0),
                                             float(sharpness)))
        return out

    def scale_yuv420(self, y, u, v=None, size=None, sharpness=0.8, out=None):
        rows, cols = y.shape
        w, h = (cols, rows) if size is None else (int(size[0]), int(size[1]))
        nv12 = v is None
        out = _planes420_empty(h, w, nv12, y.device) if out is None else tuple(out)
        self._check(self.lib.lvk_hip_scale_yuv420(self.handle, *_planes420_args((y, u, v), nv12), rows, cols, *_planes420_args(out, nv12),
                                                  h, w, 1 if nv12 else 0, float(sharpness)))
        return out

    def _px_upscale(self, sfx, src, size, out):
        out = self._px_out(sfx, src, out, (int(size[1]), int(size[0])))
        self._check(getattr(self.lib, "lvk_hip_upscale" + sfx)(self.handle, src.data_ptr(), src.stride(0), src.shape[0], src.shape[1],
                                                               out.data_ptr(), out.stride(0), out.shape[0], out.shape[1]))
        return out

    def _px_sharpen(self, sfx, src, sharpness, out):
        out = self._px_out(sfx, src, out)
        self._check(getattr(self.lib, "lvk_hip_sharpen" + sfx)(self.handle, src.data_ptr(), src.stride(0), src.shape[0], src.shape[1],
                                                               out.data_ptr(), out.stride(0), float(sharpness)))
        return out

    def upscale_gray(self, src, size, out=None):
        return self._px_upscale("_gray", src, size, out)

    def upscale_c4(self, src, size, out=None):
        return self._px_upscale("_c4", src, size, out)

    def sharpen_gray(self, src, sharpness=0.7, out=None):
        return self._px_sharpen("_gray", src, sharpness, out)

    def sharpen_c4(self, src, sharpness=0.7, out=None):
        return self._px_sharpen("_c4", src, sharpness, out)

    def mesh_solver(self, cols, rows, gen_region=(480, 270), temporal=1.0, local=20.0, max_points=4096):
        return MeshSolver(self, cols, rows, gen_region, temporal, local, max_points)

    def native_rcp(self, x):
        import torch
        x = x.contiguous()
        out = torch.empty_like(x)
        self._check(self.lib.lvk_hip_native_rcp(self.handle, x.data_ptr(), out.data_ptr(), x.numel()))
        return out

    def lens_map(self, params, rows, cols):
        import torch
        arr = (ctypes.c_double * 9)(*[float(v) for v in params])
        d = ctypes.c_void_p(); view = (ctypes.c_int * 4)()
        self._check(self.lib.lvk_hip_lens_map_create(self.handle, arr, rows, cols, ctypes.byref(d), view))
        tmp = np.zeros((rows, cols, 2), np.float32)
        self._check(self.lib.lvk_hip_download(self.handle, tmp.ctypes.data_as(ctypes.c_void_p), d, tmp.nbytes))
        self.sync()
        t = torch.from_numpy(tmp).to("cuda")
        self._check(self.lib.lvk_hip_lens_map_destroy(self.handle, d))
        return t, tuple(view)

    def warpmesh_apply_lens(self, src, mesh, params, bg=(255, 0, 255), yuv=True, out=None):
        import torch
        rows, cols = src.shape[0], src.shape[1]
        if out is None:
            out = torch.empty((rows, cols, 3), dtype=torch.uint8, device=src.device)
        m = np.ascontiguousarray(mesh, dtype=np.float32)
        ma, mp = _f32(m)
        bga, bgp = _u8x3(bg)
        arr = (ctypes.c_double * 9)(*[float(v) for v in params])
        self._check(self.lib.lvk_hip_warpmesh_apply_lens(self.handle, src.data_ptr(), src.stride(0), rows, cols, out.data_ptr(), out.stride(0),
                                                         mp, m.shape[0], m.shape[1], bgp, 1 if yuv else 0, arr))
        return out

    def lens_undistort_points(self, params, rows, cols, sx, sy, pts):
        p = np.ascontiguousarray(pts, np.float32).reshape(-1, 2)
        out = np.zeros_like(p)
        arr = (ctypes.c_double * 9)(*[float(v) for v in params])
        fp = ctypes.POINTER(ctypes.c_float)
        self._check(self.lib.lvk_hip_lens_undistort_points(self.handle, arr, rows, cols, float(sx), float(sy), p.ctypes.data_as(fp), len(p), out.ctypes.data_as(fp)))
        return out

    def draw_grid(self, frame, grid, colour, thickness=1):
        ca, cp = _u8x3(colour)
        self._check(self.lib.lvk_hip_draw_grid(self.handle, frame.data_ptr(), frame.stride(0), frame.shape[0], frame.shape[1], int(grid[0]), int(grid[1]), cp, thickness))
        return frame

    def draw_crosses(self, frame, points, colour, cross_size, thickness, scaling=(1.0, 1.0)):
        p = np.ascontiguousarray(points, np.float32).reshape(-1, 2)
        ca, cp = _u8x3(colour)
        self._check(self.lib.lvk_hip_draw_crosses(self.handle, frame.data_ptr(), frame.stride(0), frame.shape[0], frame.shape[1],
                                                  p.ctypes.data_as(ctypes.POINTER(ctypes.c_float)), len(p), float(scaling[0]), float(scaling[1]), cp,
                                                  int(cross_size), int(thickness)))
        return frame

    def fast_filter(self, prev, matched, status):
        a = np.ascontiguousarray(prev, np.float32).reshape(-1, 2); b = np.ascontiguousarray(matched, np.float32).reshape(-1, 2)
        st = np.ascontiguousarray(status, np.uint8).reshape(-1)
        oa = np.zeros_like(a); ob = np.zeros_like(b)
        fp = ctypes.POINTER(ctypes.c_float)
        m = self.lib.lvk_hip_fast_filter(self.handle, a.ctypes.data_as(fp), b.ctypes.data_as(fp), st.ctypes.data_as(ctypes.POINTER(ctypes.c_uint8)), len(a),
                                         oa.ctypes.data_as(fp), ob.ctypes.data_as(fp))
        if m < 0:
            self._check(m)
        return oa[:m], ob[:m]

    def track_chain(self, prev, matched=None, status=None, und=None, images=None, win=(11, 11), max_level=3, max_count=5, epsilon=0.01, min_eig=1e-4,
                    lens=None, threshold=3.0, region=(480, 270), full=True, full_word=None, n_word=None, separate_compact=False, host_signal=False):
        fp, bp = ctypes.POINTER(ctypes.c_float), ctypes.POINTER(ctypes.c_uint8)
        prev = np.ascontiguousarray(prev, np.float32).reshape(-1, 2)
        nb, G = len(prev), TRACK_CHAIN_GUARD
        d, r = TrackChainDesc(), TrackChainResult()
        keep = [prev]
        d.prev = prev.ctypes.data_as(fp)
        if images is None:
            matched = np.ascontiguousarray(matched, np.float32).reshape(nb, 2); status = np.ascontiguousarray(status, np.uint8).reshape(nb)
            keep += [matched, status]
            d.matched = matched.ctypes.data_as(fp); d.status = status.ctypes.data_as(bp)
            if und is not None:
                und = np.ascontiguousarray(und, np.float32).reshape(-1, 2)
                n_eff = nb if n_word is None else min(max(int(n_word), 0), nb)
                if len(und) != 2 * n_eff:
                    raise ValueError("und holds 2 x the effective count of positions (previous | matched)")
                keep.append(und)
                d.und = und.ctypes.data_as(fp)
        else:
            a, b = images
            keep += [a, b]
            d.d_prev_img = a.data_ptr(); d.prev_step = a.stride(0); d.d_next_img = b.data_ptr(); d.next_step = b.stride(0)
            d.rows, d.cols = a.shape[0], a.shape[1]
            d.win_w, d.win_h, d.max_level, d.max_count, d.epsilon, d.min_eig = win[0], win[1], max_level, max_count, float(epsilon), float(min_eig)
            if lens is not None:
                params, lrows, lcols, sx, sy = lens
                arr = (ctypes.c_double * 9)(*[float(v) for v in params])
                keep.append(arr)
                d.lens = ctypes.cast(arr, ctypes.c_void_p); d.lens_rows, d.lens_cols, d.lens_sx, d.lens_sy = int(lrows), int(lcols), float(sx), float(sy)
        d.n_bound = nb
        d.count_on_device, d.n_word = (0, 0) if n_word is None else (1, int(n_word))
        d.full = 1 if full else 0
        d.model_on_device, d.full_word = (0, 0) if full_word is None else (1, int(full_word))
        d.separate_compact = 1 if separate_compact else 0; d.host_signal = 1 if host_signal else 0
        d.threshold = float(threshold); d.region_w, d.region_h = int(region[0]), int(region[1])
        mask = np.zeros(nb, np.uint8); pairs = np.zeros((2, nb, 2), np.float32); mm = np.zeros((nb, 2), np.float32); ms = np.zeros(nb, np.uint8)
        r.mask = mask.ctypes.data_as(bp); r.pairs_dev = pairs.ctypes.data_as(fp); r.mirror_matched = mm.ctypes.data_as(fp); r.mirror_status = ms.ctypes.data_as(bp)
        out = {}
        if images is not None:
            nxt = np.zeros((nb + 2 * G, 2), np.float32); fst = np.zeros(nb + 2 * G, np.uint8); fund = np.zeros((2 * nb + 2 * G, 2), np.float32)
            r.next_pts = nxt.ctypes.data_as(fp); r.flow_status = fst.ctypes.data_as(bp); r.flow_und = fund.ctypes.data_as(fp)
            out.update(next_pts=nxt, flow_status=fst, flow_und=fund)
        self._check(self.lib.lvk_hip_track_chain(self.handle, ctypes.byref(d), ctypes.byref(r)))
        del keep
        out.update(H=np.array(r.H, np.float64).reshape(3, 3), rc=r.rc, signalled=r.signalled, count_dev=r.count_dev, count_host=r.count_host, mask=mask,
                   pairs_dev=pairs, mirror_matched=mm, mirror_status=ms)
        return out

    def warpmesh_apply_yuv420(self, src, mesh, bg=(255, 0, 255), nv12=False):
        rows, cols = src.shape[0], src.shape[1]
        out = _planes420_empty(rows, cols, nv12, src.device)
        m = np.ascontiguousarray(mesh, dtype=np.float32)
        ma, mp = _f32(m)
        bga, bgp = _u8x3(bg)
        self._check(self.lib.lvk_hip_warpmesh_apply_yuv420(self.handle, src.data_ptr(), src.stride(0), rows, cols, *_planes420_args(out, nv12), 1 if nv12 else 0,
                                                           mp, m.shape[0], m.shape[1], bgp))
        return out


class MeshSolver:

    def __init__(self, ctx, cols, rows, gen_region, temporal, local, max_points):
        self.ctx, self.cols, self.rows = ctx, cols, rows
        h = ctypes.c_void_p()
        ctx._check(ctx.lib.lvk_hip_mesh_solver_create(ctx.handle, cols, rows, float(gen_region[0]), float(gen_region[1]), float(temporal), float(local),
                                                      int(max_points), ctypes.byref(h)))
        self.handle = h

    def solve(self, tracked, matched, region=(480, 270), temporal=1.0, threshold=10.0):
        t = np.ascontiguousarray(tracked, np.float32).reshape(-1, 2); m = np.ascontiguousarray(matched, np.float32).reshape(-1, 2)
        inl = np.zeros(len(t), np.uint8); off = np.zeros((self.rows, self.cols, 2), np.float32)
        fp = ctypes.POINTER(ctypes.c_float)
        rc = self.ctx.lib.lvk_hip_mesh_solver_solve(self.handle, t.ctypes.data_as(fp), m.ctypes.data_as(fp), len(t), float(region[0]), float(region[1]),
                                                    float(temporal), float(threshold), inl.ctypes.data_as(ctypes.POINTER(ctypes.c_uint8)), off.ctypes.data_as(fp))
        if rc < 0:
            self.ctx._check(rc)
        return rc, inl, off

    def reset(self):
        self.ctx._check(self.ctx.lib.lvk_hip_mesh_solver_reset(self.handle))

    def close(self):
        if getattr(self, "handle", None):
            if getattr(self.ctx, "handle", None):
                self.ctx.lib.lvk_hip_mesh_solver_destroy(self.handle)
            self.handle = None
```

### livevisionkit_amd/csrc/lvk_hip_internal.hpp

```cpp
#pragma once

#include <hip/hip_runtime.h>
#include <cstdint>
#include <cstdio>
#include <string>
#include <vector>
#include <functional>
#include <map>
#include <set>
#include <mutex>
#include <utility>

#include "lvk_hip.h"
#include "planes420.hpp"

struct LinTabEntry { int s0, s1; float a0, a1; };
struct Lin8Entry { int s0, s1, a0, a1; };
struct AreaTabEntry { int si; float alpha; };
struct FastRegion { int x, y, w, h, threshold, active; };
constexpr int LVK_FAST_INLINE_REGIONS = 8;

constexpr int LVK_MAX_PYR_LEVELS = 8;
struct PyrLevel { const uint8_t* img; const short2* deriv; int rows, cols, step; };
struct PyrArgs { PyrLevel lv[LVK_MAX_PYR_LEVELS]; int nlevels; };

struct lvk_hip_ctx
{
    int remap_precision = LVK_REMAP_EXACT;
    int device = 0;
    int cu_count = 0;
    hipStream_t stream = nullptr;
    bool owns_stream = false;
    std::string last_error;

    static constexpr int kStageSlots = 16;
    static constexpr size_t kStageBytes = 64 * 1024;
    uint8_t* stage_host = nullptr;
    uint8_t* stage_dev = nullptr;
    hipEvent_t stage_done[kStageSlots] = {};
    int stage_next = 0;

    std::vector<hipStream_t> aux_streams;
    std::mutex aux_mutex;
    std::vector<std::pair<void*, std::function<int()>>> sync_hooks;

    std::mutex pool_mutex;
    std::multimap<size_t, void*> pool_free;
    std::map<void*, size_t> pool_sizes;
    std::set<void*> pool_cached;
    size_t pool_cached_bytes = 0;
    static constexpr size_t kPoolMaxCachedBytes = (size_t)4 << 30;

    std::vector<hipEvent_t> wait_events;

    std::map<std::tuple<int, int, int>, LinTabEntry*> lintabs;

    std::map<std::tuple<int, int, int>, Lin8Entry*> lin8tabs;

    struct AreaTabDev { int2* range = nullptr; AreaTabEntry* tab = nullptr; int max_taps = 0, span64 = 0, span4 = 0; };
    std::map<std::pair<int, int>, AreaTabDev> areatabs;
    std::map<std::pair<int, int>, int4*> enlargetabs;

    int fail(int code, const std::string& msg) { last_error = msg; if (code == LVK_HIP_ERR_RUNTIME) (void)hipGetLastError(); return code; }
};

struct lvk_device_guard
{
    int prev = -1; bool switched = false;
    explicit lvk_device_guard(const lvk_hip_ctx* ctx)
    {
        if (hipGetDevice(&prev) != hipSuccess) { (void)hipGetLastError(); prev = -1; }
        if (prev != ctx->device) switched = hipSetDevice(ctx->device) == hipSuccess;
    }
    ~lvk_device_guard() { if (switched && prev >= 0) (void)hipSetDevice(prev); }
    lvk_device_guard(const lvk_device_guard&) = delete;
    lvk_device_guard& operator=(const lvk_device_guard&) = delete;
};

#define LVK_HIP_ENTRY(ctx)                         \
    if (!(ctx)) return LVK_HIP_ERR_ARG;            \
    lvk_device_guard lvk_entry_device_guard(ctx)

#define LVK_HIP_CHECK(ctx, expr)                                                                      \
    do {                                                                                              \
        hipError_t _e = (expr);                                                                       \
        if (_e != hipSuccess)                                                                         \
        {                                                                                             \
            (void)hipGetLastError();    \
            return (ctx)->fail(LVK_HIP_ERR_RUNTIME, std::string(#expr) + ": " + hipGetErrorString(_e)); \
        }                                                                                             \
    } while (0)

#ifndef LVK_TRACKER_PRIO
#define LVK_TRACKER_PRIO 3
#endif
#define LVK_TRACKER_PRIORITY() __builtin_amdgcn_s_setprio(LVK_TRACKER_PRIO)

#if (defined(LVK_TIMELINE) || defined(LVK_RANSAC_TIMING) || defined(LVK_MESH_TIMING)) && !defined(LVK_PROBE_BUILD)
#error "instrumented build: pass -DLVK_PROBE_BUILD (scripts/variant_build.sh); never the library the tests and the bench load by default"
#endif

#ifdef LVK_TIMELINE
#define LVK_TL_SLOTS 4
#define LVK_TL_RING 8192
static __device__ unsigned lvk_tl_head[LVK_TL_SLOTS];
static __device__ unsigned long long lvk_tl_log[LVK_TL_SLOTS][LVK_TL_RING][2];
struct LvkTimelineScope
{
    int slot; bool sampled; unsigned long long t0;
    __device__ explicit LvkTimelineScope(int s) : slot(s), sampled(false), t0(0)
    {
        const unsigned total = gridDim.x * gridDim.y * gridDim.z;
        const unsigned b = (blockIdx.z * gridDim.y + blockIdx.y) * gridDim.x + blockIdx.x;
        sampled = threadIdx.x == 0 && threadIdx.y == 0 && ((b & 63u) == 63u || b == 0 || b == total - 1);
        if (sampled) t0 = (unsigned long long)wall_clock64();
    }
    __device__ ~LvkTimelineScope()
    {
        if (sampled)
        {
            const unsigned i = atomicAdd(&lvk_tl_head[slot], 1u) % LVK_TL_RING;
            lvk_tl_log[slot][i][0] = t0; lvk_tl_log[slot][i][1] = (unsigned long long)wall_clock64();
        }
    }
};
#define LVK_TL(slot) LvkTimelineScope lvk_tl_scope_(slot)
#define LVK_TL_EXPORT(unit)                                                                                     \
    extern "C" int lvk_tl_read_##unit(long long* out)                                                           \
    {                                                                                                           \
        unsigned idx[LVK_TL_SLOTS];                                                                             \
        if (hipDeviceSynchronize() != hipSuccess) return -1;                                                    \
        if (hipMemcpyFromSymbol(idx, HIP_SYMBOL(lvk_tl_head), sizeof(idx)) != hipSuccess) return -1;           \
        for (int s = 0; s < LVK_TL_SLOTS; s++) out[(size_t)s * (1 + 2 * LVK_TL_RING)] = idx[s];                 \
        for (int s = 0; s < LVK_TL_SLOTS; s++)                                                                  \
            if (hipMemcpyFromSymbol(out + (size_t)s * (1 + 2 * LVK_TL_RING) + 1, HIP_SYMBOL(lvk_tl_log), sizeof(long long) * 2 * LVK_TL_RING, \
                                    sizeof(long long) * 2 * LVK_TL_RING * s) != hipSuccess) return -1;         \
        return 0;                                                                                               \
    }
#else
#define LVK_TL(slot) do { } while (0)
#define LVK_TL_EXPORT(unit)
#endif

#define LVK_HIP_REQUIRE(ctx, cond)                                                                    \
    do { if (!(cond)) return (ctx)->fail(LVK_HIP_ERR_ARG, "pre-condition failed: " #cond); } while (0)

inline int lvk_format_channels(int format)
{
    switch (format)
    {
    case LVK_FORMAT_BGR: case LVK_FORMAT_RGB: case LVK_FORMAT_YUV: return 3;
    case LVK_FORMAT_BGRA: case LVK_FORMAT_RGBA: return 4;
    case LVK_FORMAT_GRAY: return 1;
    default: return 0;
    }
}

inline bool lvk_pitched_overlap(const void* a, int a_step, int a_rows, long long a_row_bytes, const void* b, int b_step, int b_rows, long long b_row_bytes)
{
    return yuv420::overlap(yuv420::span_of(a, a_step, a_rows, a_row_bytes), yuv420::span_of(b, b_step, b_rows, b_row_bytes));
}

int lvk_stage_params(lvk_hip_ctx* ctx, hipStream_t stream, const void* host, size_t bytes, void** d_out, int* slot = nullptr);
int lvk_stage_consumed(lvk_hip_ctx* ctx, int slot, hipStream_t stream);

int lvk_get_lintab(lvk_hip_ctx* ctx, int msize, int fsize, bool vertical, const LinTabEntry** d_out);

int lvk_get_areatab(lvk_hip_ctx* ctx, int ssize, int dsize, const int2** d_range, const AreaTabEntry** d_tab, int* max_taps = nullptr, int* span64 = nullptr, int* span4 = nullptr);

int lvk_launch_luma_area_resize(lvk_hip_ctx* ctx, const void* d_src, int src_step, int pix_stride, int channel,
                                int srows, int scols, void* d_dst, int dst_step, int drows, int dcols);
int lvk_launch_pyr_down(lvk_hip_ctx* ctx, const void* d_src, int src_step, int rows, int cols, void* d_dst, int dst_step);
int lvk_launch_scharr(lvk_hip_ctx* ctx, const void* d_src, int src_step, int rows, int cols, void* d_dst);
struct PyrArgs;
int lvk_launch_pyramid(lvk_hip_ctx* ctx, const PyrArgs& args, bool derivs = false);

int lvk_fast_workspace_bytes(int nregions, int max_rw, int max_rh, size_t* masks_bytes, size_t* scores_bytes);
int lvk_launch_fast(lvk_hip_ctx* ctx, const void* d_img, int step, int rows, int cols,
                    const FastRegion* d_regions, int nregions, int max_rw, int max_rh,
                    void* d_masks, void* d_scores, uint32_t* d_out, int cap, int* d_counts, const FastRegion* host_regions = nullptr);

struct FastInsertDesc
{
    const uint16_t* col_of; const uint32_t* row_base; const uint8_t* bucket;
    uint32_t* cell_first; void* cell_best ; int* region_count;
    const uint32_t* occ;
    const int* occ_bucket;
    int capacity; bool small_grid; int n_held, min_samples; float uniformity, homography_threshold;
    float2* pts; uint32_t* new_kp; int* result; int* d_n; int* d_full; int* counts;
};
int lvk_launch_fast_insert(lvk_hip_ctx* ctx, const void* d_img, int step, int rows, int cols, const FastRegion* host_regions, int nregions,
                           int max_rw, int max_rh, void* d_masks, void* d_scores, const FastInsertDesc& d);
bool lvk_fast_insert_fits(int cells, int nregions, int max_rw, int max_rh, int cols, int rows);
int lvk_fast_cells_reset(lvk_hip_ctx* ctx, uint32_t* d_first, void* d_best, int cells, int* d_region_count );

struct LensModel;
int lvk_pyramid_geometry(int rows, int cols, int max_level, int win_w, int win_h, int* lrows, int* lcols);
int lvk_launch_pyrlk(lvk_hip_ctx* ctx, const PyrArgs& prev, const PyrArgs& next, const float2* d_prev_pts, int n,
                     float2* d_next_pts, uint8_t* d_status, int win_w, int win_h, int max_count, double epsilon, double min_eig,
                     float2* d_prev_copy = nullptr,
                     const LensModel* lens = nullptr, double lens_sx = 0.0, double lens_sy = 0.0, float2* d_und = nullptr,
                     const int* d_n = nullptr);

struct DevicePyramid
{
    uint8_t* img_base = nullptr;
    uint8_t* deriv_base = nullptr;
    PyrArgs args{};
    int allocate(lvk_hip_ctx* ctx, int rows, int cols, int max_level, int win_w, int win_h);
    int build(lvk_hip_ctx* ctx, bool derivs = false);
    void release();
};

struct LvkHostSignal { unsigned* flag; unsigned seq; };

size_t lvk_ransac_workspace_bytes(int n);
int lvk_launch_ransac(lvk_hip_ctx* ctx, const float2* d_p1, const float2* d_p2, int n, double threshold, double region_w, double region_h,
                      bool full_homography, void* d_ws, double* d_H, int* d_ninl, uint8_t* d_mask, const int* d_n = nullptr,
                      const int* d_full = nullptr,
                      LvkHostSignal done = LvkHostSignal{nullptr, 0},
                      int lo_mode = 0);
int lvk_launch_match_compact(lvk_hip_ctx* ctx, const float2* d_prev, const float2* d_matched, const uint8_t* d_status, int n,
                             float2* d_p1, float2* d_p2, int* d_count, int* h_count, float2* h_matched, uint8_t* h_status,
                             const float2* d_und = nullptr, float region_w = 0.0f, float region_h = 0.0f,
                             const int* d_n_raw = nullptr);
constexpr int LVK_COMPACT_RANSAC_MAX = 2048;
int lvk_launch_compact_ransac(lvk_hip_ctx* ctx, const float2* d_prev, const float2* d_matched, const uint8_t* d_status, int n,
                              float2* d_p1, float2* d_p2, int* d_count, int* h_count, float2* h_matched, uint8_t* h_status,
                              const float2* d_und, float region_wf, float region_hf,
                              double threshold, double region_w, double region_h, bool full_homography, void* d_ws, double* d_H, int* d_ninl, uint8_t* d_mask,
                              const int* d_n_raw = nullptr, const int* d_full = nullptr, LvkHostSignal done = LvkHostSignal{nullptr, 0});

struct LvkTrackChain
{
    const PyrArgs* prev_pyr = nullptr; const PyrArgs* next_pyr = nullptr;
    const float2* h_pts = nullptr;
    int win_w = 0, win_h = 0, max_count = 0; double epsilon = 0.0, min_eig = 0.0;
    const LensModel* lens = nullptr; double lens_sx = 0.0, lens_sy = 0.0;
    int n = 0; const int* d_n = nullptr;
    bool full = false; const int* d_full = nullptr;
    float2* d_pts = nullptr; float2* d_matched = nullptr; uint8_t* d_status = nullptr;
    float2* d_und = nullptr;
    float2* d_p1 = nullptr; float2* d_p2 = nullptr; int* d_count = nullptr;
    int* h_count = nullptr; float2* h_matched = nullptr; uint8_t* h_status = nullptr;
    int region_w = 0, region_h = 0; double threshold = 0.0;
    bool separate_compact = false;
    bool estimate = true;
    void* d_ws = nullptr; double* h_H = nullptr; int* h_ninl = nullptr; uint8_t* h_mask = nullptr;
    LvkHostSignal done{nullptr, 0};
    void (*stage_boundary)(void* user) = nullptr; void* user = nullptr;
};
int lvk_launch_track_chain(lvk_hip_ctx* ctx, const LvkTrackChain& c);

struct LensArgs;
struct RemapLaunch
{
    hipStream_t stream = nullptr;
    int precision = LVK_REMAP_EXACT;
    const LensArgs* lens = nullptr;
    bool co_scheduled = false;
    int co_blocks_per_cu = 0;
};
int lvk_launch_remap_homography(lvk_hip_ctx* ctx, const void* d_src, int src_step, int src_rows, int src_cols,
                                void* d_dst, int dst_step, int dst_rows, int dst_cols, int off_x, int off_y,
                                const float H[9], const uint8_t bg[3], int yuv, const RemapLaunch& o);
int lvk_launch_remap_mesh(lvk_hip_ctx* ctx, const void* d_src, int src_step, int src_rows, int src_cols,
                          void* d_dst, int dst_step, const float* mesh, int mesh_rows, int mesh_cols, const uint8_t bg[3], int yuv, const RemapLaunch& o);

int lvk_launch_ingest_yuv420(lvk_hip_ctx* ctx, hipStream_t stream, const void* d_y, int y_step, const void* d_u, int u_step,
                             const void* d_v, int v_step, int nv12, int rows, int cols, void* d_dst, int dst_step);
int lvk_launch_egress_yuv420(lvk_hip_ctx* ctx, hipStream_t stream, const void* d_src, int src_step, int rows, int cols,
                             void* d_y, int y_step, void* d_u, int u_step, void* d_v, int v_step, int nv12);
int lvk_ingest_obs_check(lvk_hip_ctx* ctx, int video_format, const void* const d_planes[3], const int steps[3], int rows, int cols);
int lvk_launch_ingest_obs(lvk_hip_ctx* ctx, hipStream_t stream, int video_format, const void* const d_planes[3], const int steps[3],
                          int rows, int cols, void* d_dst, int dst_step);
int lvk_launch_egress_obs(lvk_hip_ctx* ctx, hipStream_t stream, int video_format, const void* d_src, int src_step, int rows, int cols,
                          void* const d_planes[3], const int steps[3]);


int lvk_launch_remap_map(lvk_hip_ctx* ctx, const void* d_src, int src_step, int rows, int cols,
                         void* d_dst, int dst_step, const void* d_map, int map_step, const uint8_t bg[3], int yuv, const RemapLaunch& o);

struct LensModel { double d[17]; float f[17]; int view[4]; };
struct LensModelD { double d[17]; };
__device__ __forceinline__ float2 lvk_lens_undistort_point(const LensModelD& M, double sx, double sy, float2 p)
{
    const double nfx = M.d[0], nfy = M.d[1], ncx = M.d[2], ncy = M.d[3], fx = M.d[4], fy = M.d[5], cx = M.d[6], cy = M.d[7];
    const double k1 = M.d[8], k2 = M.d[9], p1 = M.d[10], p2 = M.d[11], k3 = M.d[12];
    const double kxc = M.d[13], vxc = M.d[14], kyc = M.d[15], vyc = M.d[16];
    const double s = (double)p.x * sx, t = (double)p.y * sy;
    double u = s, v = t;
    for (int pass = 0; pass < 2; pass++)
    {
        const double s1 = s - (u * kxc + vxc), t1 = t - (v * kyc + vyc);
        const double x0 = (s1 - cx) / fx, y0 = (t1 - cy) / fy;
        double x = x0, y = y0;
        for (int j = 0; j < 5; j++)
        {
            const double r2 = x * x + y * y;
            const double icdist = 1.0 / (1 + ((k3 * r2 + k2) * r2 + k1) * r2);
            if (icdist < 0) { x = x0; y = y0; break; }
            const double dX = 2 * p1 * x * y + p2 * (r2 + 2 * x * x);
            const double dY = p1 * (r2 + 2 * y * y) + 2 * p2 * x * y;
            x = (x0 - dX) * icdist;
            y = (y0 - dY) * icdist;
        }
        u = x * nfx + ncx; v = y * nfy + ncy;
    }
    return make_float2((float)(u / sx), (float)(v / sy));
}
struct LensArgs { float f[17]; };
int lvk_lens_model_build(const lvk_camera_params& params, int rows, int cols, LensModel& out);
void lvk_lens_build_offsets(const lvk_camera_params& params, int rows, int cols, std::vector<float>& offsets, int view[4]);
int lvk_launch_lens_undistort(lvk_hip_ctx* ctx, hipStream_t stream, const LensModel& model, double sx, double sy,
                              const float2* a, int na, const float2* b, int nb, float2* out);
int lvk_launch_warpmesh_apply_lens(lvk_hip_ctx* ctx, const void* d_src, int src_step, int rows, int cols,
                                   void* d_dst, int dst_step, const float* mesh, int mesh_rows, int mesh_cols, const uint8_t bg[3], int yuv, const RemapLaunch& o);

int lvk_launch_remap_homography_gray(lvk_hip_ctx* ctx, const void* d_src, int src_step, int src_rows, int src_cols,
                                     void* d_dst, int dst_step, int dst_rows, int dst_cols, int off_x, int off_y, const float H[9], uint8_t bg, const RemapLaunch& o);
int lvk_launch_remap_mesh_gray(lvk_hip_ctx* ctx, const void* d_src, int src_step, int rows, int cols, void* d_dst, int dst_step,
                               const float* mesh, int mesh_rows, int mesh_cols, uint8_t bg, const RemapLaunch& o);
int lvk_launch_remap_map_gray(lvk_hip_ctx* ctx, const void* d_src, int src_step, int rows, int cols,
                              void* d_dst, int dst_step, const void* d_map, int map_step, uint8_t bg, const RemapLaunch& o);
int lvk_launch_warpmesh_apply_lens_gray(lvk_hip_ctx* ctx, const void* d_src, int src_step, int rows, int cols, void* d_dst, int dst_step,
                                        const float* mesh, int mesh_rows, int mesh_cols, uint8_t bg, const RemapLaunch& o);

int lvk_launch_remap_homography_c4(lvk_hip_ctx* ctx, const void* d_src, int src_step, int src_rows, int src_cols,
                                   void* d_dst, int dst_step, int dst_rows, int dst_cols, int off_x, int off_y, const float H[9], const uint8_t bg[4], const RemapLaunch& o);
int lvk_launch_remap_mesh_c4(lvk_hip_ctx* ctx, const void* d_src, int src_step, int rows, int cols, void* d_dst, int dst_step,
                             const float* mesh, int mesh_rows, int mesh_cols, const uint8_t bg[4], const RemapLaunch& o);
int lvk_launch_remap_map_c4(lvk_hip_ctx* ctx, const void* d_src, int src_step, int rows, int cols,
                            void* d_dst, int dst_step, const void* d_map, int map_step, const uint8_t bg[4], const RemapLaunch& o);
int lvk_launch_warpmesh_apply_lens_c4(lvk_hip_ctx* ctx, const void* d_src, int src_step, int rows, int cols, void* d_dst, int dst_step,
                                      const float* mesh, int mesh_rows, int mesh_cols, const uint8_t bg[4], const RemapLaunch& o);

int lvk_launch_draw_grid(lvk_hip_ctx* ctx, hipStream_t stream, void* d_dst, int dst_step, int rows, int cols, int grid_w, int grid_h,
                         const uint8_t colour[3], int thickness);
int lvk_launch_draw_crosses(lvk_hip_ctx* ctx, hipStream_t stream, void* d_dst, int dst_step, int rows, int cols, const float* pts, int n,
                            float scale_x, float scale_y, const uint8_t colour[3], int cross_size, int thickness);

int lvk_launch_upscale(lvk_hip_ctx* ctx, hipStream_t stream, const void* d_src, int src_step, int src_rows, int src_cols,
                       void* d_dst, int dst_step, int dst_rows, int dst_cols, int yuv);
int lvk_launch_sharpen(lvk_hip_ctx* ctx, hipStream_t stream, const void* d_src, int src_step, int rows, int cols,
                       void* d_dst, int dst_step, float sharpness);

struct lvk_mesh_solver_dev;
int lvk_mesh_solver_create(lvk_hip_ctx* ctx, int cols, int rows, float gen_w, float gen_h, float temporal, float local, lvk_mesh_solver_dev** out);
void lvk_mesh_solver_free(lvk_mesh_solver_dev* s);
int lvk_mesh_solver_reset(lvk_mesh_solver_dev* s, hipStream_t stream);
int lvk_mesh_solver_cols(const lvk_mesh_solver_dev* s);
int lvk_mesh_solver_rows(const lvk_mesh_solver_dev* s);
int lvk_launch_mesh_solve(lvk_mesh_solver_dev* s, hipStream_t stream, void* d_scratch , const float2* d_p1, const float2* d_p2, const int* d_count, int n_pts,
                          int min_samples, float region_w, float region_h, float temporal_now, float threshold,
                          float* h_offsets, uint8_t* h_mask, int* h_status);

int lvk_launch_warpmesh_apply_420(lvk_hip_ctx* ctx, const void* d_src, int src_step, int rows, int cols,
                                  void* o_y, int oy_step, void* o_u, int ou_step, void* o_v, int ov_step, int nv12,
                                  const float* mesh, int mesh_rows, int mesh_cols, const uint8_t bg[3], const RemapLaunch& o);
bool lvk_remap_obs_fusable(int video_format);
int lvk_launch_warpmesh_apply_obs(lvk_hip_ctx* ctx, int video_format, const void* d_src, int src_step, int rows, int cols,
                                  void* const planes[3], const int steps[3], const float* mesh, int mesh_rows, int mesh_cols, const uint8_t bg[3], const RemapLaunch& o);
```

### livevisionkit_amd/csrc/pyrlk.hip

```cpp
#include "lvk_hip_internal.hpp"

#include <climits>

namespace {

__device__ __forceinline__ int reflect101(int p, int len)
{
    if (len == 1) return 0;
    while (p < 0 || p >= len) { p = (p < 0) ? -p : 2 * (len - 1) - p; }
    return p;
}

constexpr int LK_MARGIN = 8;

__host__ __device__ inline size_t lvk_pyrlk_part_offset(int win_w, int win_h)
{
    const size_t tarea = (size_t)(win_w + 1) * (win_h + 1), area = (size_t)win_w * win_h;
    const size_t earea = (size_t)(win_w + 3) * (win_h + 3);
    const size_t jarea = (size_t)(win_w + 1 + 2 * LK_MARGIN) * (win_h + 1 + 2 * LK_MARGIN);
    return ((tarea * 4 + area * 6 + earea + jarea) + 15) & ~(size_t)15;
}

__device__ __forceinline__ int descale(int x, int n) { return (x + (1 << (n - 1))) >> n; }

__device__ __forceinline__ long long wave_sum(long long v)
{
#pragma unroll
    for (int o = 32; o >= 1; o >>= 1) v += __shfl_xor(v, o);
    return v;
}

__device__ __forceinline__ int wave_sum_i32(int v)
{
    v += __builtin_amdgcn_update_dpp(0, v, 0x111, 0xf, 0xf, true);
    v += __builtin_amdgcn_update_dpp(0, v, 0x112, 0xf, 0xf, true);
    v += __builtin_amdgcn_update_dpp(0, v, 0x114, 0xf, 0xf, true);
    v += __builtin_amdgcn_update_dpp(0, v, 0x118, 0xf, 0xf, true);
    v += __builtin_amdgcn_update_dpp(0, v, 0x142, 0xa, 0xf, false);
    v += __builtin_amdgcn_update_dpp(0, v, 0x143, 0xc, 0xf, false);
    return __builtin_amdgcn_readlane(v, 63);
}

template <int K>
__device__ __forceinline__ void wave_sums(long long (&v)[K])
{
#pragma unroll
    for (int k = 0; k < K; k++)
    {
        const int lo = (int)(v[k] & 0xffff), hi = (int)(v[k] >> 16);
        v[k] = (long long)wave_sum_i32(hi) * 65536 + (long long)wave_sum_i32(lo);
    }
}

__device__ __forceinline__ int row_sum_i32(int v)
{
    v += __builtin_amdgcn_update_dpp(0, v, 0x111, 0xf, 0xf, true);
    v += __builtin_amdgcn_update_dpp(0, v, 0x112, 0xf, 0xf, true);
    v += __builtin_amdgcn_update_dpp(0, v, 0x114, 0xf, 0xf, true);
    v += __builtin_amdgcn_update_dpp(0, v, 0x118, 0xf, 0xf, true);
    return v;
}

__device__ __forceinline__ int cross_row_sum_i32(int v)
{
    v += __builtin_amdgcn_update_dpp(0, v, 0x142, 0xa, 0xf, false);
    v += __builtin_amdgcn_update_dpp(0, v, 0x143, 0xc, 0xf, false);
    return __builtin_amdgcn_readlane(v, 63);
}

__device__ __forceinline__ void wave_sums_row32(int a, int b, long long (&v)[2])
{
    const int ra = row_sum_i32(a), rb = row_sum_i32(b);
    v[0] = (long long)cross_row_sum_i32(ra >> 16) * 65536 + (long long)cross_row_sum_i32(ra & 0xffff);
    v[1] = (long long)cross_row_sum_i32(rb >> 16) * 65536 + (long long)cross_row_sum_i32(rb & 0xffff);
}

template <int WIN>
struct LkWalk
{
    static constexpr int TRIPS = WIN > 0 ? (WIN * WIN + 63) / 64 : 1;
    static constexpr bool ROW32 = WIN > 0 && WIN * WIN <= 128;
    static_assert(!ROW32 || (long long)TRIPS * 16 * 8160 * 4080 < (1ll << 31), "a DPP row's partial of diff * Ix must fit int32");
};

__device__ __forceinline__ void bilinear_weights(float a, float b, int& w00, int& w01, int& w10, int& w11)
{
    w00 = (int)__builtin_rintf((1.f - a) * (1.f - b) * 16384.0f);
    w01 = (int)__builtin_rintf(a * (1.f - b) * 16384.0f);
    w10 = (int)__builtin_rintf((1.f - a) * b * 16384.0f);
    w11 = 16384 - w00 - w01 - w10;
}

struct LevelState
{
    float A11, A12, A22, Dinv;
    int jx0, jy0;
    int skip;
    int pad;
};

__device__ __forceinline__ void wave_lds_sync()
{
    __builtin_amdgcn_fence(__ATOMIC_RELEASE, "wavefront");
    __builtin_amdgcn_wave_barrier();
    __builtin_amdgcn_fence(__ATOMIC_ACQUIRE, "wavefront");
}

__device__ __forceinline__ int reflect101_fast(int p, int len)
{
    if (len == 1) return 0;
    p = p < 0 ? -p : p;
    p = p >= len ? 2 * (len - 1) - p : p;
    while (p < 0 || p >= len) { p = (p < 0) ? -p : 2 * (len - 1) - p; }
    return p;
}

struct WindowSrc { const uint8_t* img; int rows, cols, step, x0, y0, w, h; };

template <int CHUNK>
__device__ __forceinline__ void window_loads(uint8_t (&v)[CHUNK], const WindowSrc& s, int base, int lane)
{
    const int total = s.w * s.h;
    const float rw = 1.0f / (float)s.w;
#pragma unroll
    for (int k = 0; k < CHUNK; k++)
    {
        const int idx = min(base + k * 64 + lane, total - 1);
        int ty = (int)(((float)idx + 0.5f) * rw), tx = idx - ty * s.w;
        if (tx < 0) { ty--; tx += s.w; }
        if (tx >= s.w) { ty++; tx -= s.w; }
        v[k] = s.img[(long)reflect101_fast(s.y0 + ty, s.rows) * s.step + reflect101_fast(s.x0 + tx, s.cols)];
    }
}

template <int CHUNK>
__device__ __forceinline__ void window_stores(uint8_t* __restrict__ tile, const uint8_t (&v)[CHUNK], int total, int base, int lane)
{
#pragma unroll
    for (int k = 0; k < CHUNK; k++)
    {
        const int idx = base + k * 64 + lane;
        if (idx < total) tile[idx] = v[k];
    }
}

template <int CHUNK>
__device__ __forceinline__ void stage_window(uint8_t* __restrict__ tile, const WindowSrc& s, int lane)
{
    const int total = s.w * s.h;
    for (int base = 0; base < total; base += 64 * CHUNK)
    {
        uint8_t v[CHUNK];
        window_loads<CHUNK>(v, s, base, lane);
        window_stores<CHUNK>(tile, v, total, base, lane);
    }
}

struct __attribute__((packed, aligned(1))) LkU4B { uint32_t w; };

__device__ __forceinline__ bool window_is_interior(const WindowSrc& s)
{
    const int dpr = (s.w + 3) >> 2;
    return s.x0 >= 0 && s.y0 >= 0 && s.x0 + 4 * dpr <= s.cols && s.y0 + s.h <= s.rows;
}

template <int CHUNK>
__device__ __forceinline__ void interior_loads(uint32_t (&v)[CHUNK], const WindowSrc& s, int lane)
{
    const int dpr = (s.w + 3) >> 2, total = s.h * dpr;
    const float rd = 1.0f / (float)dpr;
    const uint8_t* origin = s.img + (long)s.y0 * s.step + s.x0;
#pragma unroll
    for (int k = 0; k < CHUNK; k++)
    {
        const int q = min(k * 64 + lane, total - 1);
        int ty = (int)(((float)q + 0.5f) * rd), tq = q - ty * dpr;
        if (tq < 0) { ty--; tq += dpr; }
        if (tq >= dpr) { ty++; tq -= dpr; }
        v[k] = reinterpret_cast<const LkU4B*>(origin + ty * s.step + 4 * tq)->w;
    }
}

template <int CHUNK>
__device__ __forceinline__ void interior_stores(uint8_t* __restrict__ tile, const uint32_t (&v)[CHUNK], const WindowSrc& s, int lane)
{
    const int dpr = (s.w + 3) >> 2, total = s.h * dpr;
    const float rd = 1.0f / (float)dpr;
#pragma unroll
    for (int k = 0; k < CHUNK; k++)
    {
        const int q = k * 64 + lane;
        int ty = (int)(((float)q + 0.5f) * rd), tq = q - ty * dpr;
        if (tq < 0) { ty--; tq += dpr; }
        if (tq >= dpr) { ty++; tq -= dpr; }
        if (q < total)
        {
            uint8_t* d = tile + ty * s.w + 4 * tq;
            const int nb = min(4, s.w - 4 * tq);
            d[0] = (uint8_t)v[k];
            if (nb > 1) d[1] = (uint8_t)(v[k] >> 8);
            if (nb > 2) d[2] = (uint8_t)(v[k] >> 16);
            if (nb > 3) d[3] = (uint8_t)(v[k] >> 24);
        }
    }
}

template <int CA, int CB, int FA, int FB>
__device__ __forceinline__ void stage_two_windows(uint8_t* __restrict__ ta, const WindowSrc& a, uint8_t* __restrict__ tb, const WindowSrc& b, bool b_valid, int lane)
{
    const bool fa = window_is_interior(a) && a.h * ((a.w + 3) >> 2) <= 64 * FA;
    const bool fb = b_valid && window_is_interior(b) && b.h * ((b.w + 3) >> 2) <= 64 * FB;
    if (fa && fb)
    {
        uint32_t va[FA], vb[FB];
        interior_loads<FA>(va, a, lane);
        interior_loads<FB>(vb, b, lane);
        interior_stores<FA>(ta, va, a, lane);
        interior_stores<FB>(tb, vb, b, lane);
        return;
    }
    const int na = a.w * a.h, nb = b_valid ? b.w * b.h : 0;
    for (int t = 0; t * 64 * CA < na || t * 64 * CB < nb; t++)
    {
        const bool do_a = t * 64 * CA < na, do_b = t * 64 * CB < nb;
        uint8_t va[CA], vb[CB];
        if (do_a) window_loads<CA>(va, a, t * 64 * CA, lane);
        if (do_b) window_loads<CB>(vb, b, t * 64 * CB, lane);
        if (do_a) window_stores<CA>(ta, va, na, t * 64 * CA, lane);
        if (do_b) window_stores<CB>(tb, vb, nb, t * 64 * CB, lane);
    }
}

template <int CB, int FB>
__device__ __forceinline__ void stage_one_window(uint8_t* __restrict__ tb, const WindowSrc& b, int lane)
{
    if (window_is_interior(b) && b.h * ((b.w + 3) >> 2) <= 64 * FB)
    {
        uint32_t vb[FB];
        interior_loads<FB>(vb, b, lane);
        interior_stores<FB>(tb, vb, b, lane);
        return;
    }
    stage_window<CB>(tb, b, lane);
}

struct LensPointArgs { LensModelD model; double sx, sy; float2* und; const int* n_dev; };
template <int WIN, bool LENS>
__global__ __launch_bounds__(64 * LVK_MAX_PYR_LEVELS)
void k_pyrlk(PyrArgs prev, PyrArgs next, const float2* __restrict__ prev_pts, float2* __restrict__ prev_copy, int n,
             float2* __restrict__ next_pts, uint8_t* __restrict__ status,
             int win_w_arg, int win_h_arg, int max_count, double epsilon_sq, float min_eig_threshold, int level_bytes_arg, LensPointArgs la)
{
    LVK_TL(0);
    LVK_TRACKER_PRIORITY();
    const int win_w = WIN ? WIN : win_w_arg, win_h = WIN ? WIN : win_h_arg;
    const int level_bytes = WIN ? (int)lvk_pyrlk_part_offset(WIN, WIN) : level_bytes_arg;
    extern __shared__ __attribute__((aligned(16))) uint8_t smem[];
    const int pt = blockIdx.x;
    if (la.n_dev) { n = min(max(*la.n_dev, 0), n); if (pt >= n) return; }
    const int lane = threadIdx.x & 63, wave = threadIdx.x >> 6;
    const int tw = win_w + 1, th = win_h + 1, area = win_w * win_h, tarea = tw * th;
    const int jw = tw + 2 * LK_MARGIN, jh = th + 2 * LK_MARGIN;
    const int ew = tw + 2, eh = th + 2;
    LevelState* states = reinterpret_cast<LevelState*>(smem + (size_t)prev.nlevels * level_bytes);
    const int py0 = lane / win_w, px0 = lane - py0 * win_w, pdy_ = 64 / win_w, pdx_ = 64 - pdy_ * win_w;
    const int lx = lane & 15, ly = lane >> 4;

    const float2 p0 = prev_pts[pt];
    if (threadIdx.x == 0 && prev_copy) prev_copy[pt] = p0;
    const float halfx = (win_w - 1) * 0.5f, halfy = (win_h - 1) * 0.5f;
    const float FLT_SCALE = 1.f / (1 << 20);
    const int top = prev.nlevels - 1;

#ifdef LVK_LK_TIMING
    long long lt[8]; int ln = 0; int iters_total = 0;
    lt[ln++] = wall_clock64();
#endif
    {
        const int level = wave;
        uint8_t* base = smem + (size_t)level * level_bytes;
        short2* dtile = reinterpret_cast<short2*>(base);
        short* Iw = reinterpret_cast<short*>(base + (size_t)tarea * 4);
        short* Ixw = Iw + area;
        short* Iyw = Ixw + area;
        uint8_t* etile = reinterpret_cast<uint8_t*>(Iyw + area);
        uint8_t* jtile = etile + ew * eh;
        const PyrLevel I = prev.lv[level];
        const PyrLevel J = next.lv[level];
        float px = p0.x * (float)(1. / (1 << level));
        float py = p0.y * (float)(1. / (1 << level));
        const float nx = px, ny = py;
        LevelState st;
        st.A11 = st.A12 = st.A22 = st.Dinv = 0.f; st.jx0 = st.jy0 = INT_MIN / 2; st.skip = 0; st.pad = 0;
        px -= halfx; py -= halfy;
        const int ipx = (int)__builtin_floorf(px), ipy = (int)__builtin_floorf(py);
        if (ipx < -win_w || ipx >= I.cols || ipy < -win_h || ipy >= I.rows) st.skip = 1;
        else
        {
            const float a = px - ipx, b = py - ipy;
            int w00, w01, w10, w11;
            bilinear_weights(a, b, w00, w01, w10, w11);
            int jx0 = (int)__builtin_floorf(nx - halfx), jy0 = (int)__builtin_floorf(ny - halfy);
            const bool j_valid = !(jx0 < -win_w || jx0 >= J.cols || jy0 < -win_h || jy0 >= J.rows);
            jx0 = j_valid ? jx0 - LK_MARGIN : INT_MIN / 2; jy0 = j_valid ? jy0 - LK_MARGIN : INT_MIN / 2;
            stage_two_windows<4, 13, 1, 4>(etile, WindowSrc{I.img, I.rows, I.cols, I.step, ipx - 1, ipy - 1, ew, eh},
                                     jtile, WindowSrc{J.img, J.rows, J.cols, J.step, jx0, jy0, jw, jh}, j_valid, lane);
            wave_lds_sync();
            for (int ty = ly; ty < th; ty += 4)
                for (int tx = lx; tx < tw; tx += 16)
                {
                    const int xx = ipx + tx, yy = ipy + ty;
                    short2 d = make_short2(0, 0);
                    if (xx >= 0 && yy >= 0 && xx < I.cols && yy < I.rows)
                    {
                        const uint8_t* r0 = etile + ty * ew + tx; const uint8_t* r1 = r0 + ew; const uint8_t* r2 = r1 + ew;
                        const int t0m = (r0[0] + r2[0]) * 3 + r1[0] * 10, t0p = (r0[2] + r2[2]) * 3 + r1[2] * 10;
                        const int t1m = r2[0] - r0[0], t1c = r2[1] - r0[1], t1p = r2[2] - r0[2];
                        d = make_short2((short)(t0p - t0m), (short)((t1p + t1m) * 3 + t1c * 10));
                    }
                    dtile[ty * tw + tx] = d;
                }
            wave_lds_sync();
            const uint8_t* tile = etile + ew + 1;
            long long sA[3] = {0, 0, 0};
            for (int p = lane, y = py0, x = px0; p < area; p += 64)
            {
                const int i00 = y * tw + x, i01 = i00 + 1, i10 = i00 + tw, i11 = i10 + 1;
                const int e00 = y * ew + x, e01 = e00 + 1, e10 = e00 + ew, e11 = e10 + 1;
                const int ival = descale(__mul24(tile[e00], w00) + __mul24(tile[e01], w01) + __mul24(tile[e10], w10) + __mul24(tile[e11], w11), 14 - 5);
                const int ixval = descale(__mul24(dtile[i00].x, w00) + __mul24(dtile[i01].x, w01) + __mul24(dtile[i10].x, w10) + __mul24(dtile[i11].x, w11), 14);
                const int iyval = descale(__mul24(dtile[i00].y, w00) + __mul24(dtile[i01].y, w01) + __mul24(dtile[i10].y, w10) + __mul24(dtile[i11].y, w11), 14);
                Iw[p] = (short)ival; Ixw[p] = (short)ixval; Iyw[p] = (short)iyval;
                sA[0] += (long long)__mul24(ixval, ixval);
                sA[1] += (long long)__mul24(ixval, iyval);
                sA[2] += (long long)__mul24(iyval, iyval);
                y += pdy_; x += pdx_; if (x >= win_w) { x -= win_w; y++; }
            }
            wave_sums<3>(sA);
            const float A11 = (float)(double)sA[0] * FLT_SCALE, A12 = (float)(double)sA[1] * FLT_SCALE, A22 = (float)(double)sA[2] * FLT_SCALE;
            const float D = A11 * A22 - A12 * A12;
            const float minEig = (A22 + A11 - __builtin_sqrtf((A11 - A22) * (A11 - A22) + 4.f * A12 * A12)) / (float)(2 * win_w * win_h);
            if (minEig < min_eig_threshold || D < 1.1920928955078125e-07f) st.skip = 1;
            else { st.A11 = A11; st.A12 = A12; st.A22 = A22; st.Dinv = 1.f / D; st.jx0 = jx0; st.jy0 = jy0; }
        }
        if (lane == 0) states[level] = st;
    }
#ifdef LVK_LK_TIMING
    lt[ln++] = wall_clock64();
#endif
    __syncthreads();
    if (wave != 0) return;
#ifdef LVK_LK_TIMING
    lt[ln++] = wall_clock64();
#endif

    float outx = 0.f, outy = 0.f;
    bool ok = true;
    constexpr int TRIPS = LkWalk<WIN>::TRIPS;
    int joff[TRIPS];
    if constexpr (LkWalk<WIN>::ROW32)
    {
#pragma unroll
        for (int r = 0; r < TRIPS; r++)
        {
            const int p = lane + 64 * r;
            joff[r] = p < area ? (p / WIN) * jw + p % WIN : py0 * jw + px0;
        }
    }
    for (int level = top; level >= 0; level--)
    {
        const PyrLevel J = next.lv[level];
        const LevelState st = states[level];
        uint8_t* base = smem + (size_t)level * level_bytes;
        const short* Iw = reinterpret_cast<const short*>(base + (size_t)tarea * 4);
        const short* Ixw = Iw + area;
        const short* Iyw = Ixw + area;
        uint8_t* jtile = base + (size_t)tarea * 4 + (size_t)area * 6 + ew * eh;
        float nx, ny;
        if (level == top) { nx = p0.x * (float)(1. / (1 << level)); ny = p0.y * (float)(1. / (1 << level)); }
        else { nx = outx * 2.f; ny = outy * 2.f; }
        outx = nx; outy = ny;
        if (st.skip)
        {
            if (level == 0) ok = false;
            continue;
        }
        const float A11 = st.A11, A12 = st.A12, A22 = st.A22, D = st.Dinv;
        int jx0 = st.jx0, jy0 = st.jy0;
        nx -= halfx; ny -= halfy;
        float pdx = 0.f, pdy = 0.f;
        int Ip[TRIPS], Ixp[TRIPS], Iyp[TRIPS];
        if constexpr (LkWalk<WIN>::ROW32)
        {
#pragma unroll
            for (int r = 0; r < TRIPS; r++)
            {
                const bool in = lane + 64 * r < area;
                const int p = in ? lane + 64 * r : lane;
                const int iv = Iw[p], ixv = Ixw[p], iyv = Iyw[p];
                Ip[r] = in ? iv : 0; Ixp[r] = in ? ixv : 0; Iyp[r] = in ? iyv : 0;
            }
        }
        for (int j = 0; j < max_count; j++)
        {
            const int inx = (int)__builtin_floorf(nx), iny = (int)__builtin_floorf(ny);
            if (inx < -win_w || inx >= J.cols || iny < -win_h || iny >= J.rows)
            {
                if (level == 0) ok = false;
                break;
            }
            const float a = nx - inx, b = ny - iny;
            int w00, w01, w10, w11;
            bilinear_weights(a, b, w00, w01, w10, w11);
            if (inx < jx0 || iny < jy0 || inx + tw > jx0 + jw || iny + th > jy0 + jh)
            {
                jx0 = inx - LK_MARGIN; jy0 = iny - LK_MARGIN;
                wave_lds_sync();
                stage_one_window<13, 4>(jtile, WindowSrc{J.img, J.rows, J.cols, J.step, jx0, jy0, jw, jh}, lane);
                wave_lds_sync();
            }
            const uint8_t* jt = jtile + (iny - jy0) * jw + (inx - jx0);
            long long sb[2] = {0, 0};
            if constexpr (LkWalk<WIN>::ROW32)
            {
                int s0 = 0, s1 = 0;
#pragma unroll
                for (int r = 0; r < TRIPS; r++)
                {
                    const int i00 = joff[r], i01 = i00 + 1, i10 = i00 + jw, i11 = i10 + 1;
                    const int diff = descale(__mul24(jt[i00], w00) + __mul24(jt[i01], w01) + __mul24(jt[i10], w10) + __mul24(jt[i11], w11), 14 - 5) - Ip[r];
                    s0 += __mul24(diff, Ixp[r]);
                    s1 += __mul24(diff, Iyp[r]);
                }
                wave_sums_row32(s0, s1, sb);
            }
            else
            {
                for (int p = lane, y = py0, x = px0; p < area; p += 64)
                {
                    const int i00 = y * jw + x, i01 = i00 + 1, i10 = i00 + jw, i11 = i10 + 1;
                    const int diff = descale(__mul24(jt[i00], w00) + __mul24(jt[i01], w01) + __mul24(jt[i10], w10) + __mul24(jt[i11], w11), 14 - 5) - Iw[p];
                    sb[0] += (long long)__mul24(diff, Ixw[p]);
                    sb[1] += (long long)__mul24(diff, Iyw[p]);
                    y += pdy_; x += pdx_; if (x >= win_w) { x -= win_w; y++; }
                }
                wave_sums<2>(sb);
            }
            const float b1 = (float)(double)sb[0] * FLT_SCALE, b2 = (float)(double)sb[1] * FLT_SCALE;
            const float dx = (A12 * b2 - A22 * b1) * D;
            const float dy = (A12 * b1 - A11 * b2) * D;
            nx += dx; ny += dy;
            outx = nx + halfx; outy = ny + halfy;
            if ((double)dx * (double)dx + (double)dy * (double)dy <= epsilon_sq) break;
            if (j > 0 && (double)__builtin_fabsf(dx + pdx) < 0.01 && (double)__builtin_fabsf(dy + pdy) < 0.01)
            {
                outx -= dx * 0.5f; outy -= dy * 0.5f;
                break;
            }
            pdx = dx; pdy = dy;
#ifdef LVK_LK_TIMING
            iters_total++;
#endif
        }
#ifdef LVK_LK_TIMING
        if (ln < 8) lt[ln++] = wall_clock64();
#endif
    }
#ifdef LVK_LK_TIMING
    if (lane == 0 && (pt == 0 || pt == 300) && n > 400)
    {
        printf("pyrlk pt %d (100 MHz ticks): phase A %lld, barrier %lld, levels", pt, lt[1] - lt[0], lt[2] - lt[1]);
        for (int k = 3; k < ln; k++) printf(" %lld", lt[k] - lt[k - 1]);
        printf(" | full iterations %d\n", iters_total);
    }
#endif
    if (lane == 0)
    {
        next_pts[pt] = make_float2(outx, outy);
        status[pt] = ok ? 1 : 0;
    }
    if (LENS && lane < 2)
    {
        const float2 q = lvk_lens_undistort_point(la.model, la.sx, la.sy, lane == 0 ? p0 : make_float2(outx, outy));
        la.und[lane == 0 ? pt : n + pt] = q;
    }
}

}

size_t lvk_pyrlk_lds_bytes(int win_w, int win_h, int nlevels)
{
    return (size_t)nlevels * lvk_pyrlk_part_offset(win_w, win_h) + (size_t)nlevels * sizeof(LevelState);
}

int lvk_launch_pyrlk(lvk_hip_ctx* ctx, const PyrArgs& prev, const PyrArgs& next, const float2* d_prev_pts, int n,
                     float2* d_next_pts, uint8_t* d_status, int win_w, int win_h, int max_count, double epsilon, double min_eig, float2* d_prev_copy,
                     const LensModel* lens, double lens_sx, double lens_sy, float2* d_und, const int* d_n)
{
    LVK_HIP_REQUIRE(ctx, prev.nlevels >= 1 && prev.nlevels == next.nlevels && prev.nlevels <= LVK_MAX_PYR_LEVELS);
    LVK_HIP_REQUIRE(ctx, win_w >= 3 && win_h >= 3 && win_w <= 31 && win_h <= 31);
    if (n <= 0) return LVK_HIP_OK;
    max_count = std::min(std::max(max_count, 0), 100);
    epsilon = std::min(std::max(epsilon, 0.), 10.);
    epsilon *= epsilon;
    const size_t lds = lvk_pyrlk_lds_bytes(win_w, win_h, prev.nlevels);
    LensPointArgs la{};
    const bool with_lens = lens != nullptr && d_und != nullptr;
    if (with_lens) { for (int i = 0; i < 17; i++) la.model.d[i] = lens->d[i]; la.sx = lens_sx; la.sy = lens_sy; la.und = d_und; }
    la.n_dev = d_n;
    auto launch = [&](auto kernel) -> int {
        if (lds > 48 * 1024)
            LVK_HIP_CHECK(ctx, hipFuncSetAttribute(reinterpret_cast<const void*>(kernel), hipFuncAttributeMaxDynamicSharedMemorySize, (int)lds));
        hipLaunchKernelGGL(kernel, dim3(n), dim3(64 * prev.nlevels), lds, ctx->stream, prev, next, d_prev_pts, d_prev_copy, n,
                           d_next_pts, d_status, win_w, win_h, max_count, epsilon, (float)min_eig, (int)lvk_pyrlk_part_offset(win_w, win_h), la);
        return LVK_HIP_OK;
    };
    int lrc;
    if (win_w == 11 && win_h == 11) lrc = with_lens ? launch(k_pyrlk<11, true>) : launch(k_pyrlk<11, false>);
    else lrc = with_lens ? launch(k_pyrlk<0, true>) : launch(k_pyrlk<0, false>);
    if (lrc != LVK_HIP_OK) return lrc;
    LVK_HIP_CHECK(ctx, hipGetLastError());
    return LVK_HIP_OK;
}

int lvk_pyramid_geometry(int rows, int cols, int max_level, int win_w, int win_h, int* lrows, int* lcols)
{
    int n = 0;
    lrows[n] = rows; lcols[n] = cols; n++;
    for (int level = 1; level <= max_level && n < LVK_MAX_PYR_LEVELS; level++)
    {
        const int r = (lrows[n - 1] + 1) / 2, c = (lcols[n - 1] + 1) / 2;
        if (c <= win_w || r <= win_h) break;
        lrows[n] = r; lcols[n] = c; n++;
    }
    return n;
}

int DevicePyramid::allocate(lvk_hip_ctx* ctx, int rows, int cols, int max_level, int win_w, int win_h)
{
    release();
    int lr[LVK_MAX_PYR_LEVELS], lc[LVK_MAX_PYR_LEVELS];
    const int n = lvk_pyramid_geometry(rows, cols, max_level, win_w, win_h, lr, lc);
    size_t img_bytes = 0, der_bytes = 0;
    for (int i = 0; i < n; i++) { img_bytes += (size_t)lr[i] * ((lc[i] + 63) & ~63); der_bytes += (size_t)lr[i] * lc[i] * 4; }
    LVK_HIP_CHECK(ctx, hipMalloc((void**)&img_base, img_bytes));
    LVK_HIP_CHECK(ctx, hipMalloc((void**)&deriv_base, der_bytes));
    uint8_t* ip = img_base; uint8_t* dp = deriv_base;
    args.nlevels = n;
    for (int i = 0; i < n; i++)
    {
        const int step = (lc[i] + 63) & ~63;
        args.lv[i].img = ip; args.lv[i].deriv = reinterpret_cast<const short2*>(dp);
        args.lv[i].rows = lr[i]; args.lv[i].cols = lc[i]; args.lv[i].step = step;
        ip += (size_t)lr[i] * step; dp += (size_t)lr[i] * lc[i] * 4;
    }
    return LVK_HIP_OK;
}

void DevicePyramid::release()
{
    if (img_base) (void)hipFree(img_base);
    if (deriv_base) (void)hipFree(deriv_base);
    img_base = deriv_base = nullptr;
    args.nlevels = 0;
}

int DevicePyramid::build(lvk_hip_ctx* ctx, bool derivs) { return lvk_launch_pyramid(ctx, args, derivs); }

extern "C" {

int lvk_hip_pyrlk(lvk_hip_ctx* ctx, const void* d_prev, int prev_step, const void* d_next, int next_step, int rows, int cols,
                  const float* prev_pts, int n, float* next_pts, uint8_t* status,
                  int win_w, int win_h, int max_level, int max_count, double epsilon, double min_eig_threshold)
{
    LVK_HIP_ENTRY(ctx);
    LVK_HIP_REQUIRE(ctx, d_prev && d_next && rows > 0 && cols > 0 && n >= 0 && (n == 0 || (prev_pts && next_pts && status)));
    DevicePyramid P, N;
    int rc;
    if ((rc = P.allocate(ctx, rows, cols, max_level, win_w, win_h)) != LVK_HIP_OK) return rc;
    if ((rc = N.allocate(ctx, rows, cols, max_level, win_w, win_h)) != LVK_HIP_OK) { P.release(); return rc; }
    float2 *d_p = nullptr, *d_n = nullptr; uint8_t* d_s = nullptr;
    auto cleanup = [&]() { P.release(); N.release(); if (d_p) (void)hipFree(d_p); if (d_n) (void)hipFree(d_n); if (d_s) (void)hipFree(d_s); };
    hipError_t e;
    if ((e = hipMemcpy2DAsync(const_cast<uint8_t*>(P.args.lv[0].img), P.args.lv[0].step, d_prev, prev_step, cols, rows, hipMemcpyDeviceToDevice, ctx->stream)) != hipSuccess ||
        (e = hipMemcpy2DAsync(const_cast<uint8_t*>(N.args.lv[0].img), N.args.lv[0].step, d_next, next_step, cols, rows, hipMemcpyDeviceToDevice, ctx->stream)) != hipSuccess)
    { cleanup(); return ctx->fail(LVK_HIP_ERR_RUNTIME, hipGetErrorString(e)); }
    if ((rc = P.build(ctx)) != LVK_HIP_OK || (rc = N.build(ctx)) != LVK_HIP_OK) { cleanup(); return rc; }
    if (n > 0)
    {
        if ((e = hipMalloc((void**)&d_p, n * sizeof(float2))) != hipSuccess || (e = hipMalloc((void**)&d_n, n * sizeof(float2))) != hipSuccess ||
            (e = hipMalloc((void**)&d_s, n)) != hipSuccess ||
            (e = hipMemcpyAsync(d_p, prev_pts, n * sizeof(float2), hipMemcpyHostToDevice, ctx->stream)) != hipSuccess)
        { cleanup(); return ctx->fail(LVK_HIP_ERR_RUNTIME, hipGetErrorString(e)); }
        if ((rc = lvk_launch_pyrlk(ctx, P.args, N.args, d_p, n, d_n, d_s, win_w, win_h, max_count, epsilon, min_eig_threshold)) != LVK_HIP_OK) { cleanup(); return rc; }
        if ((e = hipMemcpyAsync(next_pts, d_n, n * sizeof(float2), hipMemcpyDeviceToHost, ctx->stream)) != hipSuccess ||
            (e = hipMemcpyAsync(status, d_s, n, hipMemcpyDeviceToHost, ctx->stream)) != hipSuccess)
        { cleanup(); return ctx->fail(LVK_HIP_ERR_RUNTIME, hipGetErrorString(e)); }
    }
    e = hipStreamSynchronize(ctx->stream);
    cleanup();
    if (e != hipSuccess) return ctx->fail(LVK_HIP_ERR_RUNTIME, hipGetErrorString(e));
    return P.args.nlevels >= 0 ? LVK_HIP_OK : LVK_HIP_ERR_RUNTIME;
}


int lvk_hip_build_pyramid(lvk_hip_ctx* ctx, const void* d_img, int step, int rows, int cols, int max_level, int win_w, int win_h,
                          uint8_t* levels, int16_t* derivs, int* level_rows, int* level_cols)
{
    LVK_HIP_ENTRY(ctx);
    LVK_HIP_REQUIRE(ctx, d_img && levels && derivs && level_rows && level_cols && rows > 0 && cols > 0 && step >= cols);
    DevicePyramid P;
    int rc;
    if ((rc = P.allocate(ctx, rows, cols, max_level, win_w, win_h)) != LVK_HIP_OK) return rc;
    hipError_t e = hipMemcpy2DAsync(const_cast<uint8_t*>(P.args.lv[0].img), P.args.lv[0].step, d_img, step, cols, rows, hipMemcpyDeviceToDevice, ctx->stream);
    if (e == hipSuccess && (rc = P.build(ctx, true)) == LVK_HIP_OK)
    {
        size_t lo = 0, dofs = 0;
        for (int i = 0; i < P.args.nlevels && e == hipSuccess; i++)
        {
            const PyrLevel& L = P.args.lv[i];
            level_rows[i] = L.rows; level_cols[i] = L.cols;
            e = hipMemcpy2DAsync(levels + lo, L.cols, L.img, L.step, L.cols, L.rows, hipMemcpyDeviceToHost, ctx->stream);
            if (e == hipSuccess) e = hipMemcpyAsync(derivs + dofs, L.deriv, (size_t)L.rows * L.cols * 4, hipMemcpyDeviceToHost, ctx->stream);
            lo += (size_t)L.rows * L.cols; dofs += (size_t)L.rows * L.cols * 2;
        }
        if (e == hipSuccess) e = hipStreamSynchronize(ctx->stream);
    }
    const int n = P.args.nlevels;
    P.release();
    if (e != hipSuccess) return ctx->fail(LVK_HIP_ERR_RUNTIME, hipGetErrorString(e));
    return rc == LVK_HIP_OK ? n : rc;
}

}

LVK_TL_EXPORT(pyrlk)
```

### livevisionkit_amd/csrc/track_chain.hip

```cpp
#include "lvk_hip_internal.hpp"

#include <algorithm>
#include <chrono>
#include <cstring>

int lvk_launch_track_chain(lvk_hip_ctx* ctx, const LvkTrackChain& c)
{
    int rc;
    const int n = c.n;
    if (c.prev_pyr &&
        (rc = lvk_launch_pyrlk(ctx, *c.prev_pyr, *c.next_pyr, c.h_pts, n, c.d_matched, c.d_status, c.win_w, c.win_h, c.max_count, c.epsilon, c.min_eig, c.d_pts,
                               c.d_und ? c.lens : nullptr, c.lens_sx, c.lens_sy, c.d_und, c.d_n)) != LVK_HIP_OK) return rc;
    const bool fused_compact = c.estimate && !c.separate_compact && n <= LVK_COMPACT_RANSAC_MAX;
    if (!fused_compact && (rc = lvk_launch_match_compact(ctx, c.d_pts, c.d_matched, c.d_status, n, c.d_p1, c.d_p2, c.d_count, c.h_count, c.h_matched, c.h_status,
                                                         c.d_und, (float)c.region_w, (float)c.region_h, c.d_n)) != LVK_HIP_OK) return rc;
    if (c.stage_boundary) c.stage_boundary(c.user);
    if (!c.estimate) return LVK_HIP_OK;
    if (fused_compact)
        return lvk_launch_compact_ransac(ctx, c.d_pts, c.d_matched, c.d_status, n, c.d_p1, c.d_p2, c.d_count, c.h_count, c.h_matched, c.h_status,
                                         c.d_und, (float)c.region_w, (float)c.region_h,
                                         c.threshold, (double)c.region_w, (double)c.region_h, c.full, c.d_ws, c.h_H, c.h_ninl, c.h_mask, c.d_n, c.d_full, c.done);
    return lvk_launch_ransac(ctx, c.d_p1, c.d_p2, n, c.threshold, (double)c.region_w, (double)c.region_h, c.full, c.d_ws, c.h_H, c.h_ninl, c.h_mask, c.d_count, c.d_full, c.done);
}

namespace {

struct ChainBuffers
{
    std::vector<void*> dev, host;
    DevicePyramid P, N;
    template <class T> hipError_t device(T** p, size_t count) { hipError_t e = hipMalloc((void**)p, std::max<size_t>(count, 1) * sizeof(T)); if (e == hipSuccess) dev.push_back(*p); return e; }
    template <class T> hipError_t pinned(T** p, size_t count) { hipError_t e = hipHostMalloc((void**)p, std::max<size_t>(count, 1) * sizeof(T), hipHostMallocCoherent); if (e == hipSuccess) host.push_back(*p); return e; }
    ~ChainBuffers() { for (void* p : dev) (void)hipFree(p); for (void* p : host) (void)hipHostFree(p); P.release(); N.release(); }
};

}

extern "C" int lvk_hip_track_chain(lvk_hip_ctx* ctx, const lvk_track_chain_desc* d, lvk_track_chain_result* r)
{
    LVK_HIP_ENTRY(ctx);
    LVK_HIP_REQUIRE(ctx, d && r && d->prev && d->n_bound >= 1 && d->n_bound <= 4096 && d->region_w > 0 && d->region_h > 0);
    const bool flow = d->d_prev_img != nullptr;
    LVK_HIP_REQUIRE(ctx, flow ? (d->d_next_img && d->rows > 0 && d->cols > 0 && r->next_pts && r->flow_status && (!d->lens || r->flow_und))
                              : (d->matched && d->status && !d->lens));
    LVK_HIP_REQUIRE(ctx, r->mask && r->pairs_dev && r->mirror_matched && r->mirror_status);
    const int nb = d->n_bound, G = LVK_TRACK_CHAIN_GUARD;
    const int n_eff = d->count_on_device ? std::min(std::max(d->n_word, 0), nb) : nb;
    const bool with_und = flow ? d->lens != nullptr : d->und != nullptr;
    constexpr int FILL = LVK_TRACK_CHAIN_FILL;

    ChainBuffers b;
    hipStream_t st = ctx->stream;
    float2 *h_pts, *h_matched, *d_pts, *d_matched, *d_und, *d_p; uint8_t *h_status, *h_mask, *d_status; int *h_count, *h_ninl, *d_count, *d_words; double* h_H; unsigned* h_flag; void* d_ws;
    hipError_t e;
    if ((e = b.pinned(&h_pts, nb)) != hipSuccess || (e = b.pinned(&h_matched, nb)) != hipSuccess || (e = b.pinned(&h_status, nb)) != hipSuccess ||
        (e = b.pinned(&h_mask, nb)) != hipSuccess || (e = b.pinned(&h_count, 1)) != hipSuccess || (e = b.pinned(&h_ninl, 1)) != hipSuccess ||
        (e = b.pinned(&h_H, 9)) != hipSuccess || (e = b.pinned(&h_flag, 16)) != hipSuccess ||
        (e = b.device(&d_pts, nb)) != hipSuccess || (e = b.device(&d_matched, nb + 2 * G)) != hipSuccess || (e = b.device(&d_status, nb + 2 * G)) != hipSuccess ||
        (e = b.device(&d_und, 2 * nb + 2 * G)) != hipSuccess || (e = b.device(&d_p, 2 * nb)) != hipSuccess || (e = b.device(&d_count, 1)) != hipSuccess ||
        (e = b.device(&d_words, 2)) != hipSuccess || (e = hipMalloc(&d_ws, lvk_ransac_workspace_bytes(nb))) != hipSuccess)
        return ctx->fail(LVK_HIP_ERR_RUNTIME, hipGetErrorString(e));
    b.dev.push_back(d_ws);
    std::memcpy(h_pts, d->prev, (size_t)nb * sizeof(float2));
    std::memset(h_matched, FILL, (size_t)nb * sizeof(float2)); std::memset(h_status, FILL, nb); std::memset(h_mask, FILL, nb);
    *h_count = -1; *h_ninl = -1; *h_flag = 0;
    for (int q = 0; q < 9; q++) h_H[q] = 0.0;
    const int words[2] = {d->n_word, d->full_word};
    if ((e = hipMemsetAsync(d_pts, FILL, (size_t)nb * sizeof(float2), st)) != hipSuccess ||
        (e = hipMemsetAsync(d_matched, FILL, (size_t)(nb + 2 * G) * sizeof(float2), st)) != hipSuccess ||
        (e = hipMemsetAsync(d_status, FILL, (size_t)(nb + 2 * G), st)) != hipSuccess ||
        (e = hipMemsetAsync(d_und, FILL, (size_t)(2 * nb + 2 * G) * sizeof(float2), st)) != hipSuccess ||
        (e = hipMemsetAsync(d_p, FILL, (size_t)2 * nb * sizeof(float2), st)) != hipSuccess ||
        (e = hipMemsetAsync(d_count, FILL, sizeof(int), st)) != hipSuccess ||
        (e = hipMemcpyAsync(d_words, words, sizeof(words), hipMemcpyHostToDevice, st)) != hipSuccess)
        return ctx->fail(LVK_HIP_ERR_RUNTIME, hipGetErrorString(e));

    LvkTrackChain c;
    LensModel lens_model;
    if (flow)
    {
        int rc;
        if ((rc = b.P.allocate(ctx, d->rows, d->cols, d->max_level, d->win_w, d->win_h)) != LVK_HIP_OK || (rc = b.N.allocate(ctx, d->rows, d->cols, d->max_level, d->win_w, d->win_h)) != LVK_HIP_OK) return rc;
        if ((e = hipMemcpy2DAsync(const_cast<uint8_t*>(b.P.args.lv[0].img), b.P.args.lv[0].step, d->d_prev_img, d->prev_step, d->cols, d->rows, hipMemcpyDeviceToDevice, st)) != hipSuccess ||
            (e = hipMemcpy2DAsync(const_cast<uint8_t*>(b.N.args.lv[0].img), b.N.args.lv[0].step, d->d_next_img, d->next_step, d->cols, d->rows, hipMemcpyDeviceToDevice, st)) != hipSuccess)
            return ctx->fail(LVK_HIP_ERR_RUNTIME, hipGetErrorString(e));
        if ((rc = b.P.build(ctx)) != LVK_HIP_OK || (rc = b.N.build(ctx)) != LVK_HIP_OK) return rc;
        if (d->lens)
        {
            if (lvk_lens_model_build(*d->lens, d->lens_rows, d->lens_cols, lens_model) != LVK_HIP_OK) return ctx->fail(LVK_HIP_ERR_ARG, "invalid camera profile");
            c.lens = &lens_model; c.lens_sx = d->lens_sx; c.lens_sy = d->lens_sy;
        }
        c.prev_pyr = &b.P.args; c.next_pyr = &b.N.args; c.h_pts = h_pts;
        c.win_w = d->win_w; c.win_h = d->win_h; c.max_count = d->max_count; c.epsilon = d->epsilon; c.min_eig = d->min_eig;
    }
    else
    {
        if ((e = hipMemcpyAsync(d_pts, d->prev, (size_t)nb * sizeof(float2), hipMemcpyHostToDevice, st)) != hipSuccess ||
            (e = hipMemcpyAsync(d_matched + G, d->matched, (size_t)nb * sizeof(float2), hipMemcpyHostToDevice, st)) != hipSuccess ||
            (e = hipMemcpyAsync(d_status + G, d->status, (size_t)nb, hipMemcpyHostToDevice, st)) != hipSuccess ||
            (d->und && n_eff > 0 && (e = hipMemcpyAsync(d_und + G, d->und, (size_t)2 * n_eff * sizeof(float2), hipMemcpyHostToDevice, st)) != hipSuccess))
            return ctx->fail(LVK_HIP_ERR_RUNTIME, hipGetErrorString(e));
    }
    c.n = nb; c.d_n = d->count_on_device ? d_words : nullptr;
    c.full = d->full != 0; c.d_full = d->model_on_device ? d_words + 1 : nullptr;
    c.d_pts = d_pts; c.d_matched = d_matched + G; c.d_status = d_status + G; c.d_und = with_und ? d_und + G : nullptr;
    c.d_p1 = d_p; c.d_p2 = d_p + nb; c.d_count = d_count; c.h_count = h_count; c.h_matched = h_matched; c.h_status = h_status;
    c.region_w = d->region_w; c.region_h = d->region_h; c.threshold = d->threshold;
    c.separate_compact = d->separate_compact != 0;
    c.d_ws = d_ws; c.h_H = h_H; c.h_ninl = h_ninl; c.h_mask = h_mask;
    if (d->host_signal) c.done = LvkHostSignal{h_flag, 0x5EED0001u};
    int rc = lvk_launch_track_chain(ctx, c);
    if (rc != LVK_HIP_OK) { (void)hipStreamSynchronize(st); return rc; }

    r->signalled = 0;
    if (c.done.flag)
    {
        const auto t0 = std::chrono::steady_clock::now();
        for (unsigned spins = 0;; spins++)
        {
            if (__atomic_load_n(c.done.flag, __ATOMIC_ACQUIRE) == c.done.seq) { r->signalled = 1; break; }
            if ((spins & 63u) == 63u && std::chrono::steady_clock::now() - t0 > std::chrono::seconds(2)) break;
        }
    }
    if (!r->signalled)
    {
        if ((e = hipStreamSynchronize(st)) != hipSuccess) return ctx->fail(LVK_HIP_ERR_RUNTIME, hipGetErrorString(e));
        if (c.done.flag && __atomic_load_n(c.done.flag, __ATOMIC_ACQUIRE) == c.done.seq) r->signalled = 1;
    }
    std::memcpy(r->H, h_H, 9 * sizeof(double));
    const int ninl = *h_ninl;
    r->count_host = *h_count;
    std::memcpy(r->mask, h_mask, nb);
    std::memcpy(r->mirror_matched, h_matched, (size_t)nb * sizeof(float2));
    std::memcpy(r->mirror_status, h_status, nb);
    r->count_dev = -1;
    if ((e = hipMemcpyAsync(&r->count_dev, d_count, sizeof(int), hipMemcpyDeviceToHost, st)) != hipSuccess ||
        (e = hipMemcpyAsync(r->pairs_dev, d_p, (size_t)2 * nb * sizeof(float2), hipMemcpyDeviceToHost, st)) != hipSuccess ||
        (flow && ((e = hipMemcpyAsync(r->next_pts, d_matched, (size_t)(nb + 2 * G) * sizeof(float2), hipMemcpyDeviceToHost, st)) != hipSuccess ||
                  (e = hipMemcpyAsync(r->flow_status, d_status, (size_t)(nb + 2 * G), hipMemcpyDeviceToHost, st)) != hipSuccess)) ||
        (flow && r->flow_und && (e = hipMemcpyAsync(r->flow_und, d_und, (size_t)(2 * nb + 2 * G) * sizeof(float2), hipMemcpyDeviceToHost, st)) != hipSuccess) ||
        (e = hipStreamSynchronize(st)) != hipSuccess)
        return ctx->fail(LVK_HIP_ERR_RUNTIME, hipGetErrorString(e));
    if (d->host_signal && !r->signalled) return ctx->fail(LVK_HIP_ERR_RUNTIME, "the chain completed without storing its host signal word");
    r->rc = ninl >= 0 ? ninl : -10 + ninl;
    return LVK_HIP_OK;
}
```

Baseline: 9896.

## Add fewer-waves-per-point PyrLK kernel variants with batched window prefetch

Adds a template parameter so the PyrLK kernel can run with 1 or 2 waves per point instead of one wave per pyramid level. Each wave handles several levels, and the interior window loads for those levels are issued together before any LDS stores, to overlap global latency. It also adds a waves_per_eu(5) occupancy hint to all variants. The default lk_waves=0 maps to the original one-wave-per-level layout, so only the attribute changes the default path; the new variants need an explicit option.

Result: slower. 9776 (-1.2%).

```diff
diff --git a/include/lvk_hip.h b/include/lvk_hip.h
--- a/include/lvk_hip.h
+++ b/include/lvk_hip.h
@@ -330,7 +330,7 @@
 
 int lvk_hip_pyrlk(lvk_hip_ctx* ctx, const void* d_prev, int prev_step, const void* d_next, int next_step, int rows, int cols,
                   const float* prev_pts, int n, float* next_pts, uint8_t* status,
-                  int win_w, int win_h, int max_level, int max_count, double epsilon, double min_eig_threshold);
+                  int win_w, int win_h, int max_level, int max_count, double epsilon, double min_eig_threshold, int waves_per_point);
 
 int lvk_hip_estimate_global_motion(lvk_hip_ctx* ctx, const float* pts1, const float* pts2, int n, double threshold,
                                    double region_w, double region_h, int full_homography, double H[9], uint8_t* mask);
@@ -353,6 +353,7 @@
     int full, model_on_device, full_word;
     int separate_compact, host_signal;
     double threshold; int region_w, region_h;
+    int lk_waves;
 } lvk_track_chain_desc;
 typedef struct lvk_track_chain_result
 {
diff --git a/livevisionkit_amd/_native.py b/livevisionkit_amd/_native.py
--- a/livevisionkit_amd/_native.py
+++ b/livevisionkit_amd/_native.py
@@ -95,7 +95,7 @@
                                        _c.POINTER(_c.c_uint32), _c.c_int, _c.POINTER(_c.c_int)]),
     "lvk_hip_pyrlk": (_c.c_int, [_P, _P, _c.c_int, _P, _c.c_int, _c.c_int, _c.c_int, _c.POINTER(_c.c_float), _c.c_int,
                                  _c.POINTER(_c.c_float), _c.POINTER(_c.c_uint8), _c.c_int, _c.c_int, _c.c_int, _c.c_int,
-                                 _c.c_double, _c.c_double]),
+                                 _c.c_double, _c.c_double, _c.c_int]),
     "lvk_hip_ingest_yuv420": (_c.c_int, [_P, _P, _c.c_int, _P, _c.c_int, _P, _c.c_int, _c.c_int, _c.c_int, _c.c_int, _P, _c.c_int]),
     "lvk_hip_egress_yuv420": (_c.c_int, [_P, _P, _c.c_int, _c.c_int, _c.c_int, _P, _c.c_int, _P, _c.c_int, _P, _c.c_int, _c.c_int]),
     "lvk_hip_ingest_obs": (_c.c_int, [_P, _c.c_int, _P * 3, _c.c_int * 3, _c.c_int, _c.c_int, _P, _c.c_int]),
diff --git a/livevisionkit_amd/context.py b/livevisionkit_amd/context.py
--- a/livevisionkit_amd/context.py
+++ b/livevisionkit_amd/context.py
@@ -53,7 +53,8 @@
                 ("n_bound", ctypes.c_int), ("count_on_device", ctypes.c_int), ("n_word", ctypes.c_int),
                 ("full", ctypes.c_int), ("model_on_device", ctypes.c_int), ("full_word", ctypes.c_int),
                 ("separate_compact", ctypes.c_int), ("host_signal", ctypes.c_int),
-                ("threshold", ctypes.c_double), ("region_w", ctypes.c_int), ("region_h", ctypes.c_int)]
+                ("threshold", ctypes.c_double), ("region_w", ctypes.c_int), ("region_h", ctypes.c_int),
+                ("lk_waves", ctypes.c_int)]
 
 
 class TrackChainResult(ctypes.Structure):
@@ -267,7 +268,7 @@
             res.append(np.stack([e & 0xFFF, (e >> 12) & 0xFFF, e >> 24], axis=1).astype(np.int32))
         return res, counts
 
-    def pyrlk(self, prev, nxt, pts, win=(11, 11), max_level=3, max_count=5, epsilon=0.01, min_eig=1e-4):
+    def pyrlk(self, prev, nxt, pts, win=(11, 11), max_level=3, max_count=5, epsilon=0.01, min_eig=1e-4, waves=0):
         pts = np.ascontiguousarray(pts, np.float32).reshape(-1, 2)
         out = np.zeros_like(pts)
         st = np.zeros(len(pts), np.uint8)
@@ -276,7 +277,7 @@
                                            pts.ctypes.data_as(ctypes.POINTER(ctypes.c_float)), len(pts),
                                            out.ctypes.data_as(ctypes.POINTER(ctypes.c_float)),
                                            st.ctypes.data_as(ctypes.POINTER(ctypes.c_uint8)),
-                                           win[0], win[1], max_level, max_count, float(epsilon), float(min_eig)))
+                                           win[0], win[1], max_level, max_count, float(epsilon), float(min_eig), int(waves)))
         return out, st
 
     def estimate_global_motion(self, p1, p2, threshold, region=(480, 270), full_homography=True):
@@ -484,7 +485,7 @@
         return oa[:m], ob[:m]
 
     def track_chain(self, prev, matched=None, status=None, und=None, images=None, win=(11, 11), max_level=3, max_count=5, epsilon=0.01, min_eig=1e-4,
-                    lens=None, threshold=3.0, region=(480, 270), full=True, full_word=None, n_word=None, separate_compact=False, host_signal=False):
+                    lens=None, threshold=3.0, region=(480, 270), full=True, full_word=None, n_word=None, separate_compact=False, host_signal=False, lk_waves=0):
         fp, bp = ctypes.POINTER(ctypes.c_float), ctypes.POINTER(ctypes.c_uint8)
         prev = np.ascontiguousarray(prev, np.float32).reshape(-1, 2)
         nb, G = len(prev), TRACK_CHAIN_GUARD
@@ -518,6 +519,7 @@
         d.full = 1 if full else 0
         d.model_on_device, d.full_word = (0, 0) if full_word is None else (1, int(full_word))
         d.separate_compact = 1 if separate_compact else 0; d.host_signal = 1 if host_signal else 0
+        d.lk_waves = int(lk_waves)
         d.threshold = float(threshold); d.region_w, d.region_h = int(region[0]), int(region[1])
         mask = np.zeros(nb, np.uint8); pairs = np.zeros((2, nb, 2), np.float32); mm = np.zeros((nb, 2), np.float32); ms = np.zeros(nb, np.uint8)
         r.mask = mask.ctypes.data_as(bp); r.pairs_dev = pairs.ctypes.data_as(fp); r.mirror_matched = mm.ctypes.data_as(fp); r.mirror_status = ms.ctypes.data_as(bp)
diff --git a/livevisionkit_amd/csrc/lvk_hip_internal.hpp b/livevisionkit_amd/csrc/lvk_hip_internal.hpp
--- a/livevisionkit_amd/csrc/lvk_hip_internal.hpp
+++ b/livevisionkit_amd/csrc/lvk_hip_internal.hpp
@@ -200,7 +200,8 @@
                      float2* d_next_pts, uint8_t* d_status, int win_w, int win_h, int max_count, double epsilon, double min_eig,
                      float2* d_prev_copy = nullptr,
                      const LensModel* lens = nullptr, double lens_sx = 0.0, double lens_sy = 0.0, float2* d_und = nullptr,
-                     const int* d_n = nullptr);
+                     const int* d_n = nullptr,
+                     int lk_waves = 0);
 
 struct DevicePyramid
 {
@@ -236,6 +237,7 @@
     const PyrArgs* prev_pyr = nullptr; const PyrArgs* next_pyr = nullptr;
     const float2* h_pts = nullptr;
     int win_w = 0, win_h = 0, max_count = 0; double epsilon = 0.0, min_eig = 0.0;
+    int lk_waves = 0;
     const LensModel* lens = nullptr; double lens_sx = 0.0, lens_sy = 0.0;
     int n = 0; const int* d_n = nullptr;
     bool full = false; const int* d_full = nullptr;
diff --git a/livevisionkit_amd/csrc/pyrlk.hip b/livevisionkit_amd/csrc/pyrlk.hip
--- a/livevisionkit_amd/csrc/pyrlk.hip
+++ b/livevisionkit_amd/csrc/pyrlk.hip
@@ -1,6 +1,7 @@
 #include "lvk_hip_internal.hpp"
 
 #include <climits>
+#include <type_traits>
 
 namespace {
 
@@ -205,12 +206,18 @@
     }
 }
 
+template <int FA, int FB>
+__device__ __forceinline__ bool two_windows_interior(const WindowSrc& a, const WindowSrc& b, bool b_valid)
+{
+    const bool fa = window_is_interior(a) && a.h * ((a.w + 3) >> 2) <= 64 * FA;
+    const bool fb = b_valid && window_is_interior(b) && b.h * ((b.w + 3) >> 2) <= 64 * FB;
+    return fa && fb;
+}
+
 template <int CA, int CB, int FA, int FB>
 __device__ __forceinline__ void stage_two_windows(uint8_t* __restrict__ ta, const WindowSrc& a, uint8_t* __restrict__ tb, const WindowSrc& b, bool b_valid, int lane)
 {
-    const bool fa = window_is_interior(a) && a.h * ((a.w + 3) >> 2) <= 64 * FA;
-    const bool fb = b_valid && window_is_interior(b) && b.h * ((b.w + 3) >> 2) <= 64 * FB;
-    if (fa && fb)
+    if (two_windows_interior<FA, FB>(a, b, b_valid))
     {
         uint32_t va[FA], vb[FB];
         interior_loads<FA>(va, a, lane);
@@ -244,9 +251,10 @@
     stage_window<CB>(tb, b, lane);
 }
 
+constexpr int LK_WAVE_PER_LEVEL = 4;
 struct LensPointArgs { LensModelD model; double sx, sy; float2* und; const int* n_dev; };
-template <int WIN, bool LENS>
-__global__ __launch_bounds__(64 * LVK_MAX_PYR_LEVELS)
+template <int WIN, bool LENS, int WPB>
+__global__ __launch_bounds__(WPB == LK_WAVE_PER_LEVEL ? 64 * LVK_MAX_PYR_LEVELS : 64 * WPB) __attribute__((amdgpu_waves_per_eu(5)))
 void k_pyrlk(PyrArgs prev, PyrArgs next, const float2* __restrict__ prev_pts, float2* __restrict__ prev_copy, int n,
              float2* __restrict__ next_pts, uint8_t* __restrict__ status,
              int win_w_arg, int win_h_arg, int max_count, double epsilon_sq, float min_eig_threshold, int level_bytes_arg, LensPointArgs la)
@@ -258,13 +266,13 @@
     extern __shared__ __attribute__((aligned(16))) uint8_t smem[];
     const int pt = blockIdx.x;
     if (la.n_dev) { n = min(max(*la.n_dev, 0), n); if (pt >= n) return; }
-    const int lane = threadIdx.x & 63, wave = threadIdx.x >> 6;
+    const int lane = threadIdx.x & 63;
+    const int wave = WPB == 1 ? 0 : WPB == LK_WAVE_PER_LEVEL ? (int)(threadIdx.x >> 6) : __builtin_amdgcn_readfirstlane((int)(threadIdx.x >> 6));
     const int tw = win_w + 1, th = win_h + 1, area = win_w * win_h, tarea = tw * th;
     const int jw = tw + 2 * LK_MARGIN, jh = th + 2 * LK_MARGIN;
     const int ew = tw + 2, eh = th + 2;
     LevelState* states = reinterpret_cast<LevelState*>(smem + (size_t)prev.nlevels * level_bytes);
     const int py0 = lane / win_w, px0 = lane - py0 * win_w, pdy_ = 64 / win_w, pdx_ = 64 - pdy_ * win_w;
-    const int lx = lane & 15, ly = lane >> 4;
 
     const float2 p0 = prev_pts[pt];
     if (threadIdx.x == 0 && prev_copy) prev_copy[pt] = p0;
@@ -276,8 +284,11 @@
     long long lt[8]; int ln = 0; int iters_total = 0;
     lt[ln++] = wall_clock64();
 #endif
-    {
-        const int level = wave;
+    constexpr int FE = 1, FJ = 4;
+    auto prepare_level = [&](int level, bool staged, int lane_id)
+    {
+        const int lane = lane_id, lx = lane & 15, ly = lane >> 4;
+        const int py0 = lane / win_w, px0 = lane - py0 * win_w;
         uint8_t* base = smem + (size_t)level * level_bytes;
         short2* dtile = reinterpret_cast<short2*>(base);
         short* Iw = reinterpret_cast<short*>(base + (size_t)tarea * 4);
@@ -303,8 +314,9 @@
             int jx0 = (int)__builtin_floorf(nx - halfx), jy0 = (int)__builtin_floorf(ny - halfy);
             const bool j_valid = !(jx0 < -win_w || jx0 >= J.cols || jy0 < -win_h || jy0 >= J.rows);
             jx0 = j_valid ? jx0 - LK_MARGIN : INT_MIN / 2; jy0 = j_valid ? jy0 - LK_MARGIN : INT_MIN / 2;
-            stage_two_windows<4, 13, 1, 4>(etile, WindowSrc{I.img, I.rows, I.cols, I.step, ipx - 1, ipy - 1, ew, eh},
-                                     jtile, WindowSrc{J.img, J.rows, J.cols, J.step, jx0, jy0, jw, jh}, j_valid, lane);
+            if (!staged)
+                stage_two_windows<4, 13, FE, FJ>(etile, WindowSrc{I.img, I.rows, I.cols, I.step, ipx - 1, ipy - 1, ew, eh},
+                                                 jtile, WindowSrc{J.img, J.rows, J.cols, J.step, jx0, jy0, jw, jh}, j_valid, lane);
             wave_lds_sync();
             for (int ty = ly; ty < th; ty += 4)
                 for (int tx = lx; tx < tw; tx += 16)
@@ -344,11 +356,66 @@
             else { st.A11 = A11; st.A12 = A12; st.A22 = A22; st.Dinv = 1.f / D; st.jx0 = jx0; st.jy0 = jy0; }
         }
         if (lane == 0) states[level] = st;
+    };
+    if constexpr (WPB == LK_WAVE_PER_LEVEL) prepare_level(wave, false, lane);
+    else
+    {
+        constexpr int G = LK_WAVE_PER_LEVEL / WPB;
+        for (int first = wave; first < prev.nlevels; first += G * WPB)
+        {
+            uint32_t ve[G][FE], vj[G][FJ];
+            unsigned staged = 0;
+            int lane_pre = lane;
+            asm volatile("" : "+v"(lane_pre));
+            auto windows = [&](int level, WindowSrc& we, WindowSrc& wj) -> bool {
+                const PyrLevel I = prev.lv[level];
+                const PyrLevel J = next.lv[level];
+                const float nx = p0.x * (float)(1. / (1 << level)), ny = p0.y * (float)(1. / (1 << level));
+                const int ipx = (int)__builtin_floorf(nx - halfx), ipy = (int)__builtin_floorf(ny - halfy);
+                if (ipx < -win_w || ipx >= I.cols || ipy < -win_h || ipy >= I.rows) return false;
+                const bool j_valid = !(ipx >= J.cols || ipy >= J.rows);
+                we = WindowSrc{I.img, I.rows, I.cols, I.step, ipx - 1, ipy - 1, ew, eh};
+                wj = WindowSrc{J.img, J.rows, J.cols, J.step, ipx - LK_MARGIN, ipy - LK_MARGIN, jw, jh};
+                return two_windows_interior<FE, FJ>(we, wj, j_valid);
+            };
+#pragma unroll
+            for (int g = 0; g < G; g++)
+            {
+                const int level = first + g * WPB;
+                WindowSrc we, wj;
+                if (level < prev.nlevels && windows(level, we, wj))
+                {
+                    interior_loads<FE>(ve[g], we, lane_pre);
+                    interior_loads<FJ>(vj[g], wj, lane_pre);
+                    staged |= 1u << g;
+                }
+            }
+#pragma unroll
+            for (int g = 0; g < G; g++)
+            {
+                const int level = first + g * WPB;
+                WindowSrc we, wj;
+                if ((staged >> g & 1u) && windows(level, we, wj))
+                {
+                    uint8_t* etile = smem + (size_t)level * level_bytes + (size_t)tarea * 4 + (size_t)area * 6;
+                    interior_stores<FE>(etile, ve[g], we, lane_pre);
+                    interior_stores<FJ>(etile + ew * eh, vj[g], wj, lane_pre);
+                }
+            }
+#pragma unroll 1
+            for (int g = 0; g < G; g++)
+                if (first + g * WPB < prev.nlevels)
+                {
+                    int lane_id = lane;
+                    asm volatile("" : "+v"(lane_id));
+                    prepare_level(first + g * WPB, (staged >> g & 1u) != 0, lane_id);
+                }
+        }
     }
 #ifdef LVK_LK_TIMING
     lt[ln++] = wall_clock64();
 #endif
-    __syncthreads();
+    if constexpr (WPB == 1) wave_lds_sync(); else __syncthreads();
     if (wave != 0) return;
 #ifdef LVK_LK_TIMING
     lt[ln++] = wall_clock64();
@@ -495,10 +562,12 @@
 
 int lvk_launch_pyrlk(lvk_hip_ctx* ctx, const PyrArgs& prev, const PyrArgs& next, const float2* d_prev_pts, int n,
                      float2* d_next_pts, uint8_t* d_status, int win_w, int win_h, int max_count, double epsilon, double min_eig, float2* d_prev_copy,
-                     const LensModel* lens, double lens_sx, double lens_sy, float2* d_und, const int* d_n)
+                     const LensModel* lens, double lens_sx, double lens_sy, float2* d_und, const int* d_n, int lk_waves)
 {
     LVK_HIP_REQUIRE(ctx, prev.nlevels >= 1 && prev.nlevels == next.nlevels && prev.nlevels <= LVK_MAX_PYR_LEVELS);
     LVK_HIP_REQUIRE(ctx, win_w >= 3 && win_h >= 3 && win_w <= 31 && win_h <= 31);
+    if (lk_waves == 0) lk_waves = LK_WAVE_PER_LEVEL;
+    LVK_HIP_REQUIRE(ctx, lk_waves == 1 || lk_waves == 2 || lk_waves == LK_WAVE_PER_LEVEL);
     if (n <= 0) return LVK_HIP_OK;
     max_count = std::min(std::max(max_count, 0), 100);
     epsilon = std::min(std::max(epsilon, 0.), 10.);
@@ -508,16 +577,21 @@
     const bool with_lens = lens != nullptr && d_und != nullptr;
     if (with_lens) { for (int i = 0; i < 17; i++) la.model.d[i] = lens->d[i]; la.sx = lens_sx; la.sy = lens_sy; la.und = d_und; }
     la.n_dev = d_n;
+    const int waves = lk_waves == LK_WAVE_PER_LEVEL ? prev.nlevels : std::min(lk_waves, prev.nlevels);
     auto launch = [&](auto kernel) -> int {
         if (lds > 48 * 1024)
             LVK_HIP_CHECK(ctx, hipFuncSetAttribute(reinterpret_cast<const void*>(kernel), hipFuncAttributeMaxDynamicSharedMemorySize, (int)lds));
-        hipLaunchKernelGGL(kernel, dim3(n), dim3(64 * prev.nlevels), lds, ctx->stream, prev, next, d_prev_pts, d_prev_copy, n,
+        hipLaunchKernelGGL(kernel, dim3(n), dim3(64 * waves), lds, ctx->stream, prev, next, d_prev_pts, d_prev_copy, n,
                            d_next_pts, d_status, win_w, win_h, max_count, epsilon, (float)min_eig, (int)lvk_pyrlk_part_offset(win_w, win_h), la);
         return LVK_HIP_OK;
     };
-    int lrc;
-    if (win_w == 11 && win_h == 11) lrc = with_lens ? launch(k_pyrlk<11, true>) : launch(k_pyrlk<11, false>);
-    else lrc = with_lens ? launch(k_pyrlk<0, true>) : launch(k_pyrlk<0, false>);
+    auto launch_form = [&](auto wpb) -> int {
+        constexpr int W = decltype(wpb)::value;
+        if (win_w == 11 && win_h == 11) return with_lens ? launch(k_pyrlk<11, true, W>) : launch(k_pyrlk<11, false, W>);
+        return with_lens ? launch(k_pyrlk<0, true, W>) : launch(k_pyrlk<0, false, W>);
+    };
+    const int lrc = lk_waves == 1 ? launch_form(std::integral_constant<int, 1>{}) : lk_waves == 2 ? launch_form(std::integral_constant<int, 2>{})
+                                  : launch_form(std::integral_constant<int, LK_WAVE_PER_LEVEL>{});
     if (lrc != LVK_HIP_OK) return lrc;
     LVK_HIP_CHECK(ctx, hipGetLastError());
     return LVK_HIP_OK;
@@ -571,10 +645,11 @@
 
 int lvk_hip_pyrlk(lvk_hip_ctx* ctx, const void* d_prev, int prev_step, const void* d_next, int next_step, int rows, int cols,
                   const float* prev_pts, int n, float* next_pts, uint8_t* status,
-                  int win_w, int win_h, int max_level, int max_count, double epsilon, double min_eig_threshold)
+                  int win_w, int win_h, int max_level, int max_count, double epsilon, double min_eig_threshold, int waves_per_point)
 {
     LVK_HIP_ENTRY(ctx);
     LVK_HIP_REQUIRE(ctx, d_prev && d_next && rows > 0 && cols > 0 && n >= 0 && (n == 0 || (prev_pts && next_pts && status)));
+    LVK_HIP_REQUIRE(ctx, waves_per_point == 0 || waves_per_point == 1 || waves_per_point == 2 || waves_per_point == 4);
     DevicePyramid P, N;
     int rc;
     if ((rc = P.allocate(ctx, rows, cols, max_level, win_w, win_h)) != LVK_HIP_OK) return rc;
@@ -592,7 +667,8 @@
             (e = hipMalloc((void**)&d_s, n)) != hipSuccess ||
             (e = hipMemcpyAsync(d_p, prev_pts, n * sizeof(float2), hipMemcpyHostToDevice, ctx->stream)) != hipSuccess)
         { cleanup(); return ctx->fail(LVK_HIP_ERR_RUNTIME, hipGetErrorString(e)); }
-        if ((rc = lvk_launch_pyrlk(ctx, P.args, N.args, d_p, n, d_n, d_s, win_w, win_h, max_count, epsilon, min_eig_threshold)) != LVK_HIP_OK) { cleanup(); return rc; }
+        if ((rc = lvk_launch_pyrlk(ctx, P.args, N.args, d_p, n, d_n, d_s, win_w, win_h, max_count, epsilon, min_eig_threshold,
+                                   nullptr, nullptr, 0.0, 0.0, nullptr, nullptr, waves_per_point)) != LVK_HIP_OK) { cleanup(); return rc; }
         if ((e = hipMemcpyAsync(next_pts, d_n, n * sizeof(float2), hipMemcpyDeviceToHost, ctx->stream)) != hipSuccess ||
             (e = hipMemcpyAsync(status, d_s, n, hipMemcpyDeviceToHost, ctx->stream)) != hipSuccess)
         { cleanup(); return ctx->fail(LVK_HIP_ERR_RUNTIME, hipGetErrorString(e)); }
diff --git a/livevisionkit_amd/csrc/track_chain.hip b/livevisionkit_amd/csrc/track_chain.hip
--- a/livevisionkit_amd/csrc/track_chain.hip
+++ b/livevisionkit_amd/csrc/track_chain.hip
@@ -10,7 +10,7 @@
     const int n = c.n;
     if (c.prev_pyr &&
         (rc = lvk_launch_pyrlk(ctx, *c.prev_pyr, *c.next_pyr, c.h_pts, n, c.d_matched, c.d_status, c.win_w, c.win_h, c.max_count, c.epsilon, c.min_eig, c.d_pts,
-                               c.d_und ? c.lens : nullptr, c.lens_sx, c.lens_sy, c.d_und, c.d_n)) != LVK_HIP_OK) return rc;
+                               c.d_und ? c.lens : nullptr, c.lens_sx, c.lens_sy, c.d_und, c.d_n, c.lk_waves)) != LVK_HIP_OK) return rc;
     const bool fused_compact = c.estimate && !c.separate_compact && n <= LVK_COMPACT_RANSAC_MAX;
     if (!fused_compact && (rc = lvk_launch_match_compact(ctx, c.d_pts, c.d_matched, c.d_status, n, c.d_p1, c.d_p2, c.d_count, c.h_count, c.h_matched, c.h_status,
                                                          c.d_und, (float)c.region_w, (float)c.region_h, c.d_n)) != LVK_HIP_OK) return rc;
@@ -44,6 +44,7 @@
     LVK_HIP_REQUIRE(ctx, flow ? (d->d_next_img && d->rows > 0 && d->cols > 0 && r->next_pts && r->flow_status && (!d->lens || r->flow_und))
                               : (d->matched && d->status && !d->lens));
     LVK_HIP_REQUIRE(ctx, r->mask && r->pairs_dev && r->mirror_matched && r->mirror_status);
+    LVK_HIP_REQUIRE(ctx, d->lk_waves == 0 || d->lk_waves == 1 || d->lk_waves == 2 || d->lk_waves == 4);
     const int nb = d->n_bound, G = LVK_TRACK_CHAIN_GUARD;
     const int n_eff = d->count_on_device ? std::min(std::max(d->n_word, 0), nb) : nb;
     const bool with_und = flow ? d->lens != nullptr : d->und != nullptr;
@@ -92,6 +93,7 @@
         }
         c.prev_pyr = &b.P.args; c.next_pyr = &b.N.args; c.h_pts = h_pts;
         c.win_w = d->win_w; c.win_h = d->win_h; c.max_count = d->max_count; c.epsilon = d->epsilon; c.min_eig = d->min_eig;
+        c.lk_waves = d->lk_waves;
     }
     else
     {
```
